# xandercai/JSPSR

Measured on AMD Instinct MI355X. Metric: Mpixels/sec fwd+bwd, JSPSR x8 on 512^2 DEM tiles, higher is better.
Workload: dtype bf16; 1 GPU; jspsr_r8_img_msk (image+mask guided, 43.87M params), 8 x 512x512 tiles per GPU, train step (fwd + L1/L2/Sobel loss + bwd + grad all-reduce + AdamW); storage policy: bf16 activations / gradients / MFMA operands, fp32 accumulation, BatchNorm statistics, master weights and optimizer, and the generator head (affinity logits + offsets) kept as fp32 planes; tiles_per_gpu=8, tile=512, global_tiles=8, parallelism=dp1, step_mode=eager

## Files before the change

jspsr_amd/csrc/conv.hip:

```cpp
#include "conv_igemm.h"

#include <cstdlib>
#include <type_traits>

namespace {

using namespace jspsr;

constexpr int NT = 256;
constexpr int NCH = 8;
template <typename T> struct Elem;
template <> struct Elem<float> { static constexpr int EPC = 4; };
template <> struct Elem<__bf16> { static constexpr int EPC = 8; };

template <typename T> struct Mma;
template <> struct Mma<float> {
  static constexpr int BLK = 32, ROWP = 144, NE = 16, SUB = NCH / 2, SUBB = 32;
  using acc_t = f32x16;
  static __device__ __forceinline__ int frag_row(int lane) { return lane & 31; }
  static __device__ __forceinline__ int frag_chunk(int lane) { return lane >> 5; }
  static __device__ __forceinline__ int acc_row(int lane, int e) { return (e & 3) + 8 * (e >> 2) + 4 * (lane >> 5); }
  static __device__ __forceinline__ int acc_col(int lane) { return lane & 31; }
};
template <> struct Mma<__bf16> {
// ... 661 lines not shown
      if (s + 1 < M::SUB) __builtin_amdgcn_sched_group_barrier(0x100, NR, 0);
      __builtin_amdgcn_sched_group_barrier(0x008, NM, 0);
    }
  };
  auto step = [&](auto CUR, auto NXT) {
    load_b(CUR);
    const bool first_tap = (cty == 0 && ctx == 0), more = cchunk + 1 < nchunks;
    if (first_tap && more) load_patch(cchunk + 1);
    CL_STAMP(0);
    compute(CUR);
    CL_STAMP(1);
    const bool last_tap = (cty == g.nty - 1 && ctx == g.ntx - 1);
    if (last_tap && more) {
      __syncthreads();
      store_patch();
    }
    CL_STAMP(2);
    store_b(NXT, NXT);
    CL_STAMP(3);
    __syncthreads();
    CL_STAMP(4);
    if (++ctx == g.ntx) { ctx = 0; if (++cty == g.nty) { cty = 0; ++cchunk; } }
  };
  CL_STAMP3(5);
  if (KT > 0) {
    load_patch(0);
    load_b(S0{});
    load_b(S1{});
    CL_STAMP3(6);
    store_patch();
    store_b(S0{}, S0{});
  }
  CL_STAMP3(7);
  __syncthreads();
#ifdef CONVLAB_STAMPS
  CL_NOW(cl_last);
  cl_first = cl_last;
#endif
#ifdef CONVLAB_PRIO
  if ((blockIdx.x >> CONVLAB_PRIO) & 1) __builtin_amdgcn_s_setprio(1);
#endif
  int kt = 0;
  for (; kt + 1 < KT; kt += 2) {
    step(S0{}, S1{});
    step(S1{}, S0{});
  }
  if (kt < KT) step(S0{}, S1{});

#ifdef CONVLAB_STAMPS
  unsigned long long cl_loop;
  CL_NOW(cl_loop);
  cl_last = cl_loop;
#endif
  auto out_pixel = [&](int row) -> long long {
    const int y = ty0 + (row >> 4), x = tx0 + ((row + rot * (row >> 4)) & (TLW - 1));
    const int oy = y * g.oy_mul + g.oy_add, ox = x * g.ox_mul + g.ox_add;
    return (y < g.MH && x < g.MW && oy < g.OH && ox < g.OW) ? ((long long)bimg * g.OH + oy) * g.OW + ox : -1;
  };
  if (stats) {
    if constexpr (BM == 128) {
      stats_epilogue<M, MI, NI, WGM, WTM, WTN, BN>(acc, stats, smem, mt, g.Cout, n0, wm, wn, lane, out_pixel);
    } else {
      const int tty8 = (g.MH + 7) / 8;
      const int r1 = (bimg * tty8 + 2 * tyi) * ttx + txi;
      const int r2 = (2 * tyi + 1 < tty8) ? r1 + ttx : -1;
      stats_epilogue<M, MI, NI, WGM, WTM, WTN, BN>(acc, stats, smem, r1, g.Cout, n0, wm, wn, lane, out_pixel, r2);
    }
  }
  float bv[NI], sv[NI];
  int ncol[NI];
  const bool relu_first = g.relu && !g.addend, relu_last = g.relu && g.addend;
#pragma unroll
  for (int ni = 0; ni < NI; ++ni) {
    ncol[ni] = n0 + wn * WTN + ni * BLK + lc;
    bv[ni] = (bias && ncol[ni] < g.Cout) ? bias[ncol[ni]] : 0.f;
    sv[ni] = (g.scale && ncol[ni] < g.Cout) ? g.scale[ncol[ni]] : 1.f;
  }
  constexpr int OPITCH = BN * (int)sizeof(T) + 16;
  char* Os = smem;
  const bool vec_ok = (g.Cout % EPC == 0) && ((g.out_cstride * (int)sizeof(T)) % 16 == 0) &&
                      (((g.out_coff + n0) * (int)sizeof(T)) % 16 == 0) &&
                      ((reinterpret_cast<uintptr_t>(out) & 15u) == 0) &&
                      (!g.addend || (((reinterpret_cast<uintptr_t>(g.addend) & 15u) == 0) &&
                                     ((g.add_cstride * (int)sizeof(T)) % 16 == 0) && ((n0 * (int)sizeof(T)) % 16 == 0)));
  if (vec_ok) {
    constexpr int CPRO = BN * (int)sizeof(T) / 16;
    constexpr int O_IT = BM * CPRO / NTH, OB = O_IT <= 8 ? O_IT : 8;
    static_assert(BM * CPRO % NTH == 0 && O_IT % OB == 0, "epilogue rows");
    long long ooff[OB];
    uint4 areg[OB];
    uint4 zreg[OB];
    const int oy_t = ty0 * g.oy_mul + g.oy_add, ox_t = tx0 * g.ox_mul + g.ox_add, ystep = g.oy_mul * g.OW;
    const long long pix_t = ((long long)bimg * g.OH + oy_t) * g.OW + ox_t;
    const unsigned ocs = (unsigned)g.out_cstride * (unsigned)sizeof(T), acs = (unsigned)g.add_cstride * (unsigned)sizeof(T);
    const long long obase_t = pix_t * ocs, abase_t = pix_t * acs + n0 * (long long)sizeof(T);
    const unsigned zcs = (unsigned)g.red_cstride * (unsigned)sizeof(T);
    const long long zbase_t = pix_t * zcs + n0 * (long long)sizeof(T);
    const bool inside = ty0 + TLH <= g.MH && tx0 + TLW <= g.MW && oy_t + (TLH - 1) * g.oy_mul < g.OH &&
                        ox_t + (TLW - 1) * g.ox_mul < g.OW && n0 + BN <= g.Cout;
    auto plan_pieces = [&](int j0) __attribute__((always_inline)) {
#pragma unroll
      for (int j = 0; j < OB; ++j) {
        const int i = tid + (j0 + j) * NTH, row = i / CPRO, c16 = i % CPRO;
        const int dy = row >> 4, dx = (row + rot * dy) & (TLW - 1);
        const unsigned dpix = (unsigned)(dy * ystep + dx * g.ox_mul);
        bool ok = true;
        if (!inside)
          ok = ty0 + dy < g.MH && tx0 + dx < g.MW && oy_t + dy * g.oy_mul < g.OH && ox_t + dx * g.ox_mul < g.OW &&
               n0 + c16 * EPC < g.Cout;
        ooff[j] = ok ? obase_t + (long long)((unsigned long long)dpix * ocs) + c16 * 16 : -1;
        if (g.addend) {
          areg[j] = make_uint4(0, 0, 0, 0);
          if (ok)
            areg[j] = *reinterpret_cast<const uint4*>(static_cast<const char*>(g.addend) + abase_t +
                                                      (long long)((unsigned long long)dpix * acs) + c16 * 16);
        }
        if (g.red_out) {
          zreg[j] = make_uint4(0, 0, 0, 0);
          if (ok)
            zreg[j] = *reinterpret_cast<const uint4*>(static_cast<const char*>(g.red_x) + zbase_t +
                                                      (long long)((unsigned long long)dpix * zcs) + c16 * 16);
        }
      }
    };
    float rs1[EPC], rs2[EPC], rpa[EPC], rpb[EPC], rpi[EPC], rpm[EPC];
    if (g.red_out) {
      static_assert(NTH % CPRO == 0, "a thread's pieces share their channels");
      const int cc = n0 + (tid % CPRO) * EPC;
#pragma unroll
      for (int e2 = 0; e2 < EPC; ++e2) {
        const bool in_c = cc + e2 < g.Cout;
        rs1[e2] = rs2[e2] = 0.f;
        rpa[e2] = in_c ? g.red_par[cc + e2] : 0.f;
        rpb[e2] = in_c ? g.red_par[g.Cout + cc + e2] : 0.f;
        rpi[e2] = in_c ? g.red_par[2 * g.Cout + cc + e2] : 0.f;
        rpm[e2] = in_c ? g.red_par[3 * g.Cout + cc + e2] : 0.f;
      }
    }
    plan_pieces(0);
#pragma unroll
    for (int mi = 0; mi < MI; ++mi)
#pragma unroll
      for (int e = 0; e < M::NE; ++e) {
        const int row = wm * WTM + mi * BLK + M::acc_row(lane, e);
#pragma unroll
        for (int ni = 0; ni < NI; ++ni) {
          float v = acc[mi][ni][e] * sv[ni] + bv[ni];
          if (relu_first) v = fmaxf(v, 0.f);
          *reinterpret_cast<T*>(Os + row * OPITCH + (wn * WTN + ni * BLK + lc) * (int)sizeof(T)) = (T)v;
        }
      }
    CL_STAMP3(0);
    __syncthreads();
    CL_STAMP3(1);
    char* const obase = reinterpret_cast<char*>(out + g.out_coff + n0);
#pragma unroll
    for (int j0 = 0; j0 < O_IT; j0 += OB) {
      if (j0) plan_pieces(j0);
      uint4 ov[OB];
#pragma unroll
      for (int j = 0; j < OB; ++j) {
        const int i = tid + (j0 + j) * NTH, row = i / CPRO, c16 = i % CPRO;
        ov[j] = *reinterpret_cast<const uint4*>(Os + row * OPITCH + c16 * 16);
      }
      CL_STAMP3(2);
#pragma unroll
      for (int j = 0; j < OB; ++j) {
        if (ooff[j] < 0) continue;
        uint4 v = ov[j];
        if (g.addend) v = add_packed<T>(v, areg[j]);
        if (relu_last) v = relu_packed<T>(v);
        *reinterpret_cast<uint4*>(obase + ooff[j]) = v;
        if (g.red_out) {
          float dv[EPC], zv[EPC];
          unpack_chunk<T>(v, dv);
          unpack_chunk<T>(zreg[j], zv);
#pragma unroll
          for (int e2 = 0; e2 < EPC; ++e2) {
            const float dz = rpa[e2] * zv[e2] + rpb[e2] > 0.f ? dv[e2] : 0.f;
            rs1[e2] += dz;
            rs2[e2] += dz * (zv[e2] * rpi[e2] + rpm[e2]);
          }
        }
      }
    }
    if (g.red_out) {
      __syncthreads();
      float* red = reinterpret_cast<float*>(smem);
#pragma unroll
      for (int e2 = 0; e2 < EPC; ++e2) {
        red[tid * 2 * EPC + e2] = rs1[e2];
        red[tid * 2 * EPC + EPC + e2] = rs2[e2];
      }
      __syncthreads();
      int r1 = mt, r2 = -1;
      if constexpr (BM != 128) {
        const int tty8 = (g.MH + 7) / 8;
        r1 = (bimg * tty8 + 2 * tyi) * ttx + txi;
        r2 = (2 * tyi + 1 < tty8) ? r1 + ttx : -1;
      }
      for (int i = tid; i < 2 * BN; i += NTH) {
        const int which = i / BN, col = i % BN;
        if (n0 + col >= g.Cout) continue;
        const int cg_ = col / EPC, e2 = col % EPC;
        float tsum = 0.f;
        for (int k2 = 0; k2 < NTH / CPRO; ++k2) tsum += red[(cg_ + CPRO * k2) * 2 * EPC + which * EPC + e2];
        g.red_out[((size_t)r1 * 2 + which) * g.Cout + n0 + col] = tsum;
        if (r2 >= 0) g.red_out[((size_t)r2 * 2 + which) * g.Cout + n0 + col] = 0.f;
      }
    }
  } else {
#pragma unroll
    for (int mi = 0; mi < MI; ++mi)
#pragma unroll
      for (int e = 0; e < M::NE; ++e) {
        const int row = wm * WTM + mi * BLK + M::acc_row(lane, e);
        const long long opix = out_pixel(row);
        if (opix < 0) continue;
        T* orow = out + opix * g.out_cstride + g.out_coff;
#pragma unroll
        for (int ni = 0; ni < NI; ++ni) {
          if (ncol[ni] >= g.Cout) continue;
          float v = acc[mi][ni][e] * sv[ni] + bv[ni];
          if (relu_first) v = fmaxf(v, 0.f);
          if (g.addend) v = (float)(T)v + (float)static_cast<const T*>(g.addend)[opix * g.add_cstride + ncol[ni]];
          if (relu_last) v = fmaxf(v, 0.f);
          orow[ncol[ni]] = (T)v;
        }
      }
  }
#ifdef CONVLAB_STAMPS
  if ((tid & 63) == 0) {
    unsigned long long end_;
    CL_NOW(end_);
    unsigned long long* o = convlab_stamp + (size_t)((blockIdx.x * (NTH / 64) + (tid >> 6)) % CONVLAB_SLOTS) * 16;
    for (int i = 0; i < 4; ++i) o[i] = cl_stamp[i] + (i == 3 ? cl_stamp[4] : 0);
    o[4] = cl_first - cl_entry;
    o[5] = cl_loop - cl_first;
    o[6] = end_ - cl_loop;
    for (int i = 5; i < 8; ++i) o[3 + i] = cl_stamp[i];
    o[11] = cl_stamp[4];
    o[7] = (unsigned long long)KT;
  }
#endif
}

template <typename T, int BM, int BN, int WGM, int WGN>
int launch_patch(const void* in, const void* wgt, const float* bias, void* out, float* stats, const ConvGeom& g, hipStream_t s) {
  constexpr int NTH = 64 * WGM * WGN, TLW = 16, TLH = BM / TLW, MAXPIX = patch_it(BM, NTH) * NTH / NCH;
  const long long nblk = (long long)g.B * ((g.MH + TLH - 1) / TLH) * ((g.MW + TLW - 1) / TLW) * ((g.Cout + BN - 1) / BN);
  if (nblk > 0x7fffffffLL || (long long)TLH * g.oy_mul * g.OW + (long long)TLW * g.ox_mul > 0x7fffffffLL)
    return fail(JSPSR_EINVAL, "conv: grid too large");
  constexpr int ROWB = Mma<T>::ROWP;
  const size_t lds_stage = (size_t)MAXPIX * ROWB + 2 * BN * ROWB, lds_out = (size_t)BM * (BN * sizeof(T) + 16);
  const size_t lds = lds_stage > lds_out ? lds_stage : lds_out;
  ConvGeom gk = g;
  gk.fd_ntn = make_fastdiv((unsigned)((g.Cout + BN - 1) / BN));
  gk.fd_ttx = make_fastdiv((unsigned)((g.MW + TLW - 1) / TLW));
  gk.fd_tty = make_fastdiv((unsigned)((g.MH + TLH - 1) / TLH));
  auto kern = conv_patch_kernel<T, BM, BN, WGM, WGN>;
  static bool attr_set = false;
  if (!attr_set) {
    (void)hipFuncSetAttribute(reinterpret_cast<const void*>(kern), hipFuncAttributeMaxDynamicSharedMemorySize, (int)lds);
    attr_set = true;
  }
  hipLaunchKernelGGL(kern, dim3((unsigned)nblk), dim3(NTH), lds, s, static_cast<const T*>(in), static_cast<const T*>(wgt),
                     bias, static_cast<T*>(out), stats, gk);
  return check_launch(BM == 256 ? (BN == 64 ? "conv_patch_16x16" : "conv_patch_16x16x128") : "conv_patch");
}

template <typename T, int BM, int BN, int WGM, int WGN, int NBUF>
int launch_cfg(const void* in, const void* wgt, const float* bias, void* out, float* stats, const ConvGeom& g, hipStream_t s) {
  if ((long long)g.B * g.MH * g.MW <= 0) return JSPSR_OK;
  constexpr int TLW = 16, TLH = BM / TLW;
  const long long nblk = (long long)g.B * ((g.MH + TLH - 1) / TLH) * ((g.MW + TLW - 1) / TLW) * ((g.Cout + BN - 1) / BN);
  if (nblk > 0x7fffffffLL) return fail(JSPSR_EINVAL, "conv: grid too large");
  constexpr int ROWB = IgemmMma<T, NBUF>::ROWP;
  const size_t lds_stage = NBUF * (BM + BN) * ROWB, lds_out = (size_t)BM * (BN * sizeof(T) + 16);
  const size_t lds = lds_stage > lds_out ? lds_stage : lds_out;
  constexpr int BK = NCH * Elem<T>::EPC;
  static bool attr_set = false;
  if (!attr_set) {
    (void)hipFuncSetAttribute(reinterpret_cast<const void*>(conv_igemm_kernel<T, BM, BN, WGM, WGN, true, NBUF>),
                              hipFuncAttributeMaxDynamicSharedMemorySize, (int)lds);
    (void)hipFuncSetAttribute(reinterpret_cast<const void*>(conv_igemm_kernel<T, BM, BN, WGM, WGN, false, NBUF>),
                              hipFuncAttributeMaxDynamicSharedMemorySize, (int)lds);
    attr_set = true;
  }
  if (g.Cin % BK == 0)
    hipLaunchKernelGGL((conv_igemm_kernel<T, BM, BN, WGM, WGN, true, NBUF>), dim3((unsigned)nblk), dim3(NT), lds, s,
                       static_cast<const T*>(in), static_cast<const T*>(wgt), bias, static_cast<T*>(out), stats, g);
  else
    hipLaunchKernelGGL((conv_igemm_kernel<T, BM, BN, WGM, WGN, false, NBUF>), dim3((unsigned)nblk), dim3(NT), lds, s,
                       static_cast<const T*>(in), static_cast<const T*>(wgt), bias, static_cast<T*>(out), stats, g);
  return check_launch("conv_igemm");
}

template <typename T>
int launch(const void* in, const void* wgt, const float* bias, void* out, float* stats, const ConvGeom& g, hipStream_t s) {
  static const int no_patch = [] { const char* e = getenv("JSPSR_CONV_NOPATCH"); return e ? atoi(e) : 0; }();
  constexpr int BKT = NCH * Elem<T>::EPC;
  if constexpr (sizeof(T) == 2)
  {
    if (conv64_resident_ok(g, in, wgt, bias, out)) return launch_conv64_resident(in, wgt, bias, out, stats, g, s);
    if (conv128_resident_ok(g, in, wgt, bias, out)) return launch_conv128_resident(in, wgt, bias, out, stats, g, s);
  }
  if ((!no_patch || g.in_affine) && g.iy_mul == 1 && g.ix_mul == 1 && g.nty >= 1 && g.ntx >= 1 && g.nty <= 3 && g.ntx <= 3 &&
      g.nty * g.ntx > 1 && g.Cin % BKT == 0 && (long long)(g.IW + 20) * 12 * g.in_cstride * (long long)sizeof(T) < 0xE0000000LL) {
    static const int tall = [] { const char* e = getenv("JSPSR_CONV_TALL"); return e ? atoi(e) : 1; }();
    const long long tiles16 = (long long)g.B * ((g.MH + 15) / 16) * ((g.MW + 15) / 16);
    if (g.Cout > 64) {
      if (tall == 2 && tiles16 * ((g.Cout + 127) / 128) >= 512) return launch_patch<T, 256, 128, 4, 2>(in, wgt, bias, out, stats, g, s);
      if (tall && tall != 4 && tiles16 * ((g.Cout + 63) / 64) >= 1024) return launch_patch<T, 256, 64, 4, 1>(in, wgt, bias, out, stats, g, s);
      return launch_patch<T, 128, 128, 2, 2>(in, wgt, bias, out, stats, g, s);
    }
    if (g.Cout > 32) {
      if (tall && tiles16 >= 1024) return launch_patch<T, 256, 64, 4, 1>(in, wgt, bias, out, stats, g, s);
      return launch_patch<T, 128, 64, 2, 2>(in, wgt, bias, out, stats, g, s);
    }
    return launch_patch<T, 128, 32, 4, 1>(in, wgt, bias, out, stats, g, s);
  }
  if (g.red_out) return fail(JSPSR_EINVAL, "conv2d_dgrad: the fused BatchNorm-backward reduce needs the patch kernel (jspsr_conv2d_dgrad_reduce_ok)");
  if (g.in_affine) return fail(JSPSR_EINVAL, "conv2d_forward: in_affine needs the patch kernel (stride 1, 2..9 taps, Cin a multiple of %d): ask jspsr_conv2d_in_affine_ok first", BKT);
  static const int nbuf_env = [] { const char* e = getenv("JSPSR_CONV_NBUF"); return e ? atoi(e) : 0; }();
  const int nbuf_narrow = nbuf_env ? nbuf_env : ((long long)g.nty * g.ntx * g.Cin <= 1152 ? 1 : 2);
  if (g.Cout > 64) return launch_cfg<T, 128, 128, 2, 2, 2>(in, wgt, bias, out, stats, g, s);
  if (nbuf_narrow == 2) {
    if (g.Cout > 32) return launch_cfg<T, 128, 64, 2, 2, 2>(in, wgt, bias, out, stats, g, s);
    return launch_cfg<T, 128, 32, 4, 1, 2>(in, wgt, bias, out, stats, g, s);
  }
  if (g.Cout > 32) return launch_cfg<T, 128, 64, 2, 2, 1>(in, wgt, bias, out, stats, g, s);
  return launch_cfg<T, 128, 32, 4, 1, 1>(in, wgt, bias, out, stats, g, s);
}

int check_common(int dtype, const void* a, const void* w, const void* o, int cin, int cs_in, int co_in,
                 int cs_out, int co_out, int cout, const char* what) {
  if (dtype != JSPSR_F32 && dtype != JSPSR_BF16) return fail(JSPSR_EINVAL, "%s: dtype must be JSPSR_F32 or JSPSR_BF16", what);
  if (!a || !w || !o) return fail(JSPSR_EINVAL, "%s: null pointer", what);
  const int epc = dtype == JSPSR_F32 ? 4 : 8;
  if (cin <= 0 || cin % epc || cs_in % epc || co_in % epc || cs_in < co_in + cin)
    return fail(JSPSR_EINVAL, "%s: gathered channels (C=%d pitch=%d off=%d) must be multiples of %d", what, cin, cs_in, co_in, epc);
  if (cout <= 0 || cs_out < co_out + cout) return fail(JSPSR_EINVAL, "%s: bad output channel slice", what);
  if (!aligned16(a) || !aligned16(w)) return fail(JSPSR_EALIGN, "%s: input/weight pointers must be 16-byte aligned", what);
  return JSPSR_OK;
}

template <typename T>
__global__ void pack_weight_kernel(const float* __restrict__ w, T* __restrict__ out, int O, int I, int KH, int KW,
                                   int mode, int Cpad, long long total) {
  for (long long idx = blockIdx.x * (long long)blockDim.x + threadIdx.x; idx < total;
       idx += (long long)gridDim.x * blockDim.x) {
    const int c = (int)(idx % Cpad);
    long long r = idx / Cpad;
    const int kx = (int)(r % KW); r /= KW;
    const int ky = (int)(r % KH); r /= KH;
    const int n = (int)r;
    float v = 0.f;
    if (mode == 0) { if (c < I) v = w[(((size_t)n * I + c) * KH + ky) * KW + kx]; }
    else           { if (c < O) v = w[(((size_t)c * I + n) * KH + ky) * KW + kx]; }
    out[idx] = (T)v;
  }
}

constexpr int PACK_CHUNK = 2048;
__global__ __launch_bounds__(256) void pack_weights_multi_kernel(const jspsr_pack_desc* __restrict__ descs, int n) {
  int lo = 0, hi = n - 1;
  const long long b = blockIdx.x;
  while (lo < hi) {
    const int mid = (lo + hi + 1) >> 1;
    if (descs[mid].start <= b) lo = mid; else hi = mid - 1;
  }
  const jspsr_pack_desc d = descs[lo];
  const long long l0 = (b - d.start) * PACK_CHUNK;
  const float* __restrict__ w = d.w;
#pragma unroll
  for (int k = 0; k < PACK_CHUNK / 256; ++k) {
    const long long l = l0 + k * 256 + threadIdx.x;
    if (l >= d.total) break;
    const int c = (int)(l % d.c_pad);
    long long r = l / d.c_pad;
    const int kx = (int)(r % d.KW); r /= d.KW;
    const int ky = (int)(r % d.KH); r /= d.KH;
    const int nn = (int)r;
    float v = 0.f;
    if (d.mode == 0) { if (c < d.I) v = w[(((size_t)nn * d.I + c) * d.KH + ky) * d.KW + kx]; }
    else             { if (c < d.O) v = w[(((size_t)c * d.I + nn) * d.KH + ky) * d.KW + kx]; }
    if (d.dtype == JSPSR_F32) static_cast<float*>(d.out)[l] = v;
    else static_cast<__bf16*>(d.out)[l] = (__bf16)v;
  }
}

}

extern "C" int jspsr_pack_weights_multi(const jspsr_pack_desc* descs, int n, long long total_blocks, jspsr_stream_t stream) {
  if (!descs || n <= 0 || total_blocks <= 0 || total_blocks > 0x7fffffffLL) return fail(JSPSR_EINVAL, "pack_weights_multi: bad arguments");
  hipLaunchKernelGGL(pack_weights_multi_kernel, dim3((unsigned)total_blocks), dim3(256), 0, static_cast<hipStream_t>(stream), descs, n);
  return check_launch("pack_weights_multi");
}

extern "C" int jspsr_pack_chunk(void) { return PACK_CHUNK; }

extern "C" int jspsr_pack_weight(int dtype, const float* w, void* packed, int O, int I, int KH, int KW,
                                 int mode, int c_pad, jspsr_stream_t stream) {
  if (!w || !packed || O <= 0 || I <= 0 || KH <= 0 || KW <= 0 || (mode != 0 && mode != 1))
    return fail(JSPSR_EINVAL, "pack_weight: bad arguments");
  const int C = mode == 0 ? I : O, N = mode == 0 ? O : I;
  if (c_pad < C) return fail(JSPSR_EINVAL, "pack_weight: c_pad %d < %d", c_pad, C);
  const long long total = (long long)N * KH * KW * c_pad;
  const int blocks = (int)((total + 255) / 256 < 4096 ? (total + 255) / 256 : 4096);
  hipStream_t s = static_cast<hipStream_t>(stream);
  if (dtype == JSPSR_F32)
    hipLaunchKernelGGL(pack_weight_kernel<float>, dim3(blocks), dim3(256), 0, s, w, static_cast<float*>(packed), O, I, KH, KW, mode, c_pad, total);
  else if (dtype == JSPSR_BF16)
    hipLaunchKernelGGL(pack_weight_kernel<__bf16>, dim3(blocks), dim3(256), 0, s, w, static_cast<__bf16*>(packed), O, I, KH, KW, mode, c_pad, total);
  else
    return fail(JSPSR_EINVAL, "pack_weight: bad dtype");
  return check_launch("pack_weight");
}

extern "C" int jspsr_conv2d_stats_rows(int B, int OH, int OW) {
  if (B <= 0 || OH <= 0 || OW <= 0) return 0;
  return B * ((OH + 7) / 8) * ((OW + 15) / 16);
}

extern "C" int jspsr_conv2d_forward(int dtype, const void* in, const void* wpack, const float* bias, void* out,
                                    int B, int IH, int IW, int Cin, int in_cstride, int in_coff, int Cout,
                                    int out_cstride, int out_coff, int KH, int KW, int stride, int pad, int relu,
                                    float* stats, const float* scale, const void* addend, int add_cstride,
                                    const float* in_affine, int in_relu, jspsr_stream_t stream) {
  if (int e = check_common(dtype, in, wpack, out, Cin, in_cstride, in_coff, out_cstride, out_coff, Cout, "conv2d_forward")) return e;
  if (in_affine && !aligned16(in_affine)) return fail(JSPSR_EALIGN, "conv2d_forward: in_affine must be 16-byte aligned");
  if (addend && add_cstride < Cout) return fail(JSPSR_EINVAL, "conv2d_forward: addend pitch %d < %d channels", add_cstride, Cout);
  if (B <= 0 || IH <= 0 || IW <= 0 || KH <= 0 || KW <= 0 || stride <= 0 || pad < 0)
    return fail(JSPSR_EINVAL, "conv2d_forward: bad geometry");
  ConvGeom g{};
  g.B = B; g.IH = IH; g.IW = IW; g.Cin = Cin;
  g.OH = (IH + 2 * pad - KH) / stride + 1;
  g.OW = (IW + 2 * pad - KW) / stride + 1;
  if (g.OH <= 0 || g.OW <= 0) return fail(JSPSR_EINVAL, "conv2d_forward: empty output");
  g.Cout = Cout; g.in_cstride = in_cstride; g.in_coff = in_coff; g.out_cstride = out_cstride; g.out_coff = out_coff;
  g.MH = g.OH; g.MW = g.OW;
  g.iy_mul = stride; g.iy_add = -pad; g.ix_mul = stride; g.ix_add = -pad; g.sign = 1;
  g.nty = KH; g.ntx = KW; g.ky0 = 0; g.kx0 = 0; g.kstep = 1; g.KH = KH; g.KW = KW;
  g.oy_mul = 1; g.oy_add = 0; g.ox_mul = 1; g.ox_add = 0; g.relu = relu;
  g.accumulate = getenv("JSPSR_CONV_NOXCD") ? 1 : 0;
  hipStream_t s = static_cast<hipStream_t>(stream);
  if (stats && (bias || relu || scale || addend))
    return fail(JSPSR_EINVAL, "conv2d_forward: statistics are taken from the raw accumulators (no bias / scale / addend / ReLU)");
  g.scale = scale; g.addend = addend; g.add_cstride = add_cstride;
  g.in_affine = in_affine; g.in_relu = in_relu;
  return dtype == JSPSR_F32 ? launch<float>(in, wpack, bias, out, stats, g, s) : launch<__bf16>(in, wpack, bias, out, stats, g, s);
}

extern "C" int jspsr_conv2d_in_affine_ok(int dtype, int Cin, int KH, int KW, int stride) {
  const int bk = NCH * (dtype == JSPSR_F32 ? 4 : 8);
  return (dtype == JSPSR_F32 || dtype == JSPSR_BF16) && stride == 1 && KH >= 1 && KW >= 1 && KH <= 3 && KW <= 3 && KH * KW > 1 &&
         Cin > 0 && Cin % bk == 0;
}

extern "C" int jspsr_conv2d_dgrad_reduce_ok(int dtype, int B, int IH, int IW, int Cg, int Cin, int KH, int KW, int stride, int pad) {
  if (dtype != JSPSR_F32 && dtype != JSPSR_BF16) return 0;
  static const int off = [] { const char* e = getenv("JSPSR_BN_REDUCE_FUSE"); return e && atoi(e) == 0; }();
  if (off) return 0;
  const int epc = dtype == JSPSR_F32 ? 4 : 8, bkt = NCH * epc;
  if (KH != 3 || KW != 3 || stride != 1 || pad != 1 || Cg <= 0 || Cg % bkt || Cin <= 0 || Cin % epc || B <= 0 || IH <= 0 || IW <= 0) return 0;
  static const int no_patch = [] { const char* e = getenv("JSPSR_CONV_NOPATCH"); return e ? atoi(e) : 0; }();
  if (no_patch) return 0;
  if (dtype == JSPSR_BF16 && Cg == 64 && Cin == 64) {
    static const int resident = [] { const char* e = getenv("JSPSR_CONV_RESIDENT"); return e ? atoi(e) : 1; }();
    static const int min_tiles = [] { const char* e = getenv("JSPSR_CONV_RESIDENT_MIN"); return e ? atoi(e) : 512; }();
    if (resident && (long long)B * ((IH + 15) / 16) * ((IW + 15) / 16) >= min_tiles) return 0;
  }
  return 1;
}

extern "C" int jspsr_conv2d_dgrad(int dtype, const void* gout, const void* wpack_t, const float* bias, void* gin,
                                  int B, int OH, int OW, int Cg, int g_cstride, int g_coff, int IH, int IW,
                                  int Cin, int in_cstride, int in_coff, int KH, int KW, int stride, int pad,
                                  int relu, const void* addend, int add_cstride, const float* scale,
                                  const void* red_x, int red_cstride, const float* red_par, float* red_out,
                                  jspsr_stream_t stream) {
  if (int e = check_common(dtype, gout, wpack_t, gin, Cg, g_cstride, g_coff, in_cstride, in_coff, Cin, "conv2d_dgrad")) return e;
  if (addend && add_cstride < Cin) return fail(JSPSR_EINVAL, "conv2d_dgrad: addend pitch %d < %d channels", add_cstride, Cin);
  if (red_out) {
    if (!red_x || !red_par || !jspsr_conv2d_dgrad_reduce_ok(dtype, B, IH, IW, Cg, Cin, KH, KW, stride, pad))
      return fail(JSPSR_EINVAL, "conv2d_dgrad: the fused BatchNorm-backward reduce needs jspsr_conv2d_dgrad_reduce_ok(...) != 0");
    const int epc = dtype == JSPSR_F32 ? 4 : 8;
    if (red_cstride < Cin || red_cstride % epc || in_cstride % epc || in_coff % epc || !aligned16(red_x) || !aligned16(gin) ||
        (addend && (!aligned16(addend) || add_cstride % epc)))
      return fail(JSPSR_EALIGN, "conv2d_dgrad: fused reduce needs 16-byte pieces (pitches / offsets multiples of %d, aligned tensors)", epc);
  }
  if (B <= 0 || OH <= 0 || OW <= 0 || IH <= 0 || IW <= 0 || KH <= 0 || KW <= 0 || stride <= 0 || pad < 0)
    return fail(JSPSR_EINVAL, "conv2d_dgrad: bad geometry");
  hipStream_t s = static_cast<hipStream_t>(stream);
  for (int py = 0; py < stride; ++py)
    for (int px = 0; px < stride; ++px) {
      ConvGeom g{};
      g.B = B; g.IH = OH; g.IW = OW; g.Cin = Cg;
      g.OH = IH; g.OW = IW; g.Cout = Cin;
      g.in_cstride = g_cstride; g.in_coff = g_coff; g.out_cstride = in_cstride; g.out_coff = in_coff;
      g.MH = (IH - py + stride - 1) / stride;
      g.MW = (IW - px + stride - 1) / stride;
      if (g.MH <= 0 || g.MW <= 0) continue;
      g.ky0 = (py + pad) % stride; g.kx0 = (px + pad) % stride; g.kstep = stride;
      g.nty = g.ky0 < KH ? (KH - g.ky0 + stride - 1) / stride : 0;
      g.ntx = g.kx0 < KW ? (KW - g.kx0 + stride - 1) / stride : 0;
      if (g.nty == 0 || g.ntx == 0) g.nty = g.ntx = 0;
      g.iy_mul = 1; g.iy_add = (py + pad - g.ky0) / stride; g.ix_mul = 1; g.ix_add = (px + pad - g.kx0) / stride;
      g.sign = -1; g.KH = KH; g.KW = KW;
      g.oy_mul = stride; g.oy_add = py; g.ox_mul = stride; g.ox_add = px; g.relu = relu;
      g.addend = addend; g.add_cstride = add_cstride; g.scale = scale;
      g.red_x = red_x; g.red_cstride = red_cstride; g.red_par = red_par; g.red_out = red_out;
      const int e = dtype == JSPSR_F32 ? launch<float>(gout, wpack_t, bias, gin, nullptr, g, s)
                                       : launch<__bf16>(gout, wpack_t, bias, gin, nullptr, g, s);
      if (e) return e;
    }
  return JSPSR_OK;
}

#ifdef CONVLAB_STAMPS
extern "C" int jspsr_lab_conv_stamps(unsigned long long* out16, int reset) {
  static unsigned long long host[CONVLAB_SLOTS * 16];
  if (hipMemcpyFromSymbol(host, HIP_SYMBOL(convlab_stamp), sizeof(host)) != hipSuccess) return 1;
  for (int i = 0; i < 16; ++i) out16[i] = 0;
  for (int r = 0; r < CONVLAB_SLOTS; ++r)
    if (host[r * 16 + 7]) { for (int i = 0; i < 16; ++i) out16[i] += host[r * 16 + i]; }
  if (reset) { for (size_t i = 0; i < sizeof(host) / 8; ++i) host[i] = 0; if (hipMemcpyToSymbol(HIP_SYMBOL(convlab_stamp), host, sizeof(host)) != hipSuccess) return 1; }
  return 0;
}
#endif
```

jspsr_amd/csrc/conv128.hip:

```cpp
#include "conv_igemm.h"

#include <atomic>

#include <cstdlib>
#include <type_traits>

namespace {

using namespace jspsr;

constexpr int Q_NTH = 256;
constexpr int Q_TH = 8, Q_TW = 16;
constexpr int Q_PH = Q_TH + 2, Q_PW = Q_TW + 2, Q_NPIX = Q_PH * Q_PW;
constexpr int Q_PIXB = 256;
constexpr int Q_PATCHB = Q_NPIX * Q_PIXB;
constexpr int Q_PIECES = Q_PATCHB / 1024;
static_assert(Q_PIECES * 1024 == Q_PATCHB, "whole pieces");
constexpr int Q_NP = (Q_PIECES + 3) / 4;
constexpr int Q_BUF1 = 65536;
constexpr int Q_XCHB = 16384;
constexpr int Q_OFF_RED = Q_PATCHB + Q_XCHB;
static_assert(Q_OFF_RED + 2048 <= Q_BUF1, "the first 64 KiB hold patch 0, inbox 0 and the fold");
constexpr int Q_OFF_RUN = Q_OFF_RED + 2048;
static_assert(Q_OFF_RUN + 16 <= Q_BUF1, "run starts inside the first 64 KiB");
constexpr int Q_RUN = 4;
constexpr int Q_OFF_DUMP = Q_BUF1 + Q_PATCHB + 3 * Q_XCHB;
constexpr int Q_OFF_PAR = Q_OFF_DUMP + 1024;
constexpr int Q_LDS = Q_OFF_PAR + 1024;
static_assert(Q_LDS <= 163840, "LDS of one CU");
constexpr int Q_ROWS4 = 4 * Q_PW * Q_PIXB;
#ifndef K2Q_LA
#define K2Q_LA 4
#endif
#ifndef K2Q_DMA_MODE
#define K2Q_DMA_MODE 1
#endif
#ifndef K2Q_LD_EVERY
#define K2Q_LD_EVERY 9
#endif
#ifndef K2Q_LD_DIST
#define K2Q_LD_DIST 27
#endif
#ifndef K2Q_DMA_EVERY
#define K2Q_DMA_EVERY 6
#endif
constexpr int Q_NK = 144, Q_LAH = K2Q_LA;

__device__ __forceinline__ int inbox_off(int wave) { return wave == 0 ? Q_PATCHB : Q_BUF1 + Q_PATCHB + (wave - 1) * Q_XCHB; }

template <int SH, int N>
__device__ __forceinline__ void row_sum(float (&v)[N]) {
#pragma unroll
  for (int c = 0; c < N; ++c)
    v[c] += __builtin_bit_cast(float, __builtin_amdgcn_update_dpp(0, __builtin_bit_cast(int, v[c]), 0x120 + SH, 0xf, 0xf, false));
}

template <int B, int E, typename F>
__device__ __forceinline__ void static_for(F&& f) {
  if constexpr (B < E) {
    f(std::integral_constant<int, B>{});
    static_for<B + 1, E>(f);
  }
}

template <bool FIRST, bool WA>
__device__ __forceinline__ void mfma4(f32x4& c0, f32x4& c1, f32x4& c2, f32x4& c3, const i32x4& w0, const i32x4& w1, const i32x4& w2,
                                      const i32x4& w3, const i32x4& b) {
#define K2Q_MFMA4(OUT, CC, WC)                                                                                           \
  asm volatile("v_mfma_f32_16x16x32_bf16 %0, %4, %8, " CC "0\n\tv_mfma_f32_16x16x32_bf16 %1, %5, %8, " CC "1\n\t"        \
               "v_mfma_f32_16x16x32_bf16 %2, %6, %8, " CC "2\n\tv_mfma_f32_16x16x32_bf16 %3, %7, %8, " CC "3"             \
               : OUT(c0), OUT(c1), OUT(c2), OUT(c3) : WC(w0), WC(w1), WC(w2), WC(w3), "v"(b))
  if constexpr (FIRST) {
    if constexpr (WA)
      asm volatile("v_mfma_f32_16x16x32_bf16 %0, %4, %8, 0\n\tv_mfma_f32_16x16x32_bf16 %1, %5, %8, 0\n\t"
                   "v_mfma_f32_16x16x32_bf16 %2, %6, %8, 0\n\tv_mfma_f32_16x16x32_bf16 %3, %7, %8, 0"
                   : "=&v"(c0), "=&v"(c1), "=&v"(c2), "=&v"(c3) : "a"(w0), "a"(w1), "a"(w2), "a"(w3), "v"(b));
    else
      asm volatile("v_mfma_f32_16x16x32_bf16 %0, %4, %8, 0\n\tv_mfma_f32_16x16x32_bf16 %1, %5, %8, 0\n\t"
                   "v_mfma_f32_16x16x32_bf16 %2, %6, %8, 0\n\tv_mfma_f32_16x16x32_bf16 %3, %7, %8, 0"
                   : "=&v"(c0), "=&v"(c1), "=&v"(c2), "=&v"(c3) : "v"(w0), "v"(w1), "v"(w2), "v"(w3), "v"(b));
  } else {
    if constexpr (WA) K2Q_MFMA4("+v", "%", "a");
    else K2Q_MFMA4("+v", "%", "v");
  }
#undef K2Q_MFMA4
}

typedef const i32x4 __attribute__((address_space(3)))* lds_frag_t;

struct QTile { int bimg, tyi, txi; };
struct QSrc { i32x4 desc; __amdgpu_buffer_rsrc_t rsrc; int oy0, ox0; bool interior; };

template <int SIGN, int MODE, int KH>
__device__ __forceinline__ void conv128_body(const __bf16* __restrict__ in, const __bf16* __restrict__ wgt, const float* __restrict__ bias,
                                             __bf16* __restrict__ out, float* __restrict__ stats, const ConvGeom& g, int ntiles, unsigned* __restrict__ ticket, char* smem) {
  constexpr bool STATS = MODE == 1, AFFINE = MODE == 2;
  const int tid = threadIdx.x, wave = __builtin_amdgcn_readfirstlane(tid >> 6), lane = tid & 63;
  const int cg = wave & 1;
  const int n = lane & 15, q = lane >> 4;
  const int ttx = (g.MW + Q_TW - 1) / Q_TW, tty = (g.MH + Q_TH - 1) / Q_TH;
  const int G = gridDim.x;
  const unsigned lds0 = (unsigned)(size_t)(lptr_t)smem;
  if (lds0 != 0) __builtin_trap();
  const int v = xcd_contiguous(blockIdx.x, G);

  i32x4 breg[9][2][4];
#pragma unroll
  for (int cb = 0; cb < 4; ++cb) {
    const int ch = 64 * cg + 32 * (cb >> 1) + 8 * (n >> 2) + 4 * (cb & 1) + (n & 3);
    const char* wrow = reinterpret_cast<const char*>(wgt) + (size_t)ch * (9 * 128 * 2) + (64 * KH + 8 * q) * 2;
#pragma unroll
    for (int t = 0; t < 9; ++t)
#pragma unroll
      for (int s = 0; s < 2; ++s) breg[t][s][cb] = *reinterpret_cast<const i32x4*>(wrow + t * 256 + s * 64);
  }

  const int dGx = G % ttx, dGy = (G / ttx) % tty, dGb = G / (ttx * tty);
  auto advance = [&](QTile c) {
    c.txi += dGx;
    int carry = c.txi >= ttx;
    c.txi -= carry ? ttx : 0;
    c.tyi += dGy + carry;
    carry = c.tyi >= tty;
    c.tyi -= carry ? tty : 0;
    c.bimg += dGb + carry;
    return c;
  };

  const int pix_bytes = g.in_cstride * 2;
  constexpr int back = SIGN < 0 ? 2 : 0;
  auto patch_src = [&](QTile tc, bool more) {
    QSrc p;
    p.oy0 = tc.tyi * Q_TH + g.iy_add - back;
    p.ox0 = tc.txi * Q_TW + g.ix_add - back;
    const long long opix0 = ((long long)tc.bimg * g.IH + p.oy0) * g.IW + p.ox0;
    const unsigned long long b64 = reinterpret_cast<unsigned long long>(in) + (opix0 * g.in_cstride + g.in_coff) * 2;
    p.desc = i32x4{(int)(unsigned)b64, (int)((unsigned)(b64 >> 32) & 0xffffu), more ? (int)0xFFFFFF00u : 0, 0x00020000};
    p.interior = p.oy0 >= 0 && p.ox0 >= 0 && p.oy0 + Q_PH <= g.IH && p.ox0 + Q_PW <= g.IW;
    p.rsrc = __builtin_amdgcn_make_buffer_rsrc(reinterpret_cast<char*>(b64), 0, more ? 0xFFFFFF00u : 0u, 0x00020000);
    return p;
  };
  const int p0lane = 4 * wave + q;
  const unsigned swz16 = (unsigned)((n ^ (2 * (p0lane & 7))) << 4);
  unsigned dsrc[Q_NP];
#pragma unroll
  for (int i = 0; i < Q_NP; ++i) {
    const int P = p0lane + 16 * i, py = P / Q_PW, px = P - py * Q_PW;
    dsrc[i] = (unsigned)((py * g.IW + px) * pix_bytes) + swz16;
  }
  struct PieceXY { int py, px; unsigned off; };
  auto piece_xy = [&](int i) __attribute__((always_inline)) {
    int p0 = p0lane;
    asm volatile("" : "+v"(p0));
    const int P = p0 + 16 * i;
    PieceXY c;
    c.py = (int)(__umul24(P, 3641) >> 16);
    unsigned t = __umul24(c.py, Q_PW);
    asm("" : "+v"(t));
    c.px = P - (int)t;
    unsigned t2 = __umul24(c.py, g.IW);
    asm("" : "+v"(t2));
    c.off = t2 + (unsigned)c.px;
    return c;
  };
  auto piece_src = [&](const QSrc& p, const PieceXY& c) __attribute__((always_inline)) {
    unsigned b = __umul24(c.off, pix_bytes);
    asm("" : "+v"(b));
    unsigned src = b + swz16;
    src = (unsigned)(p.oy0 + c.py) < (unsigned)g.IH ? src : 0xFFFFFFF0u;
    src = (unsigned)(p.ox0 + c.px) < (unsigned)g.IW ? src : 0xFFFFFFF0u;
    return src;
  };
  auto piece_dst = [&](unsigned bufoff, int i) __attribute__((always_inline)) {
#ifdef K2Q_LAB_TODUMP
    return (unsigned)Q_OFF_DUMP;
#endif
    return (wave + 4 * i < Q_PIECES) ? bufoff + (unsigned)(wave + 4 * i) * 1024u : (unsigned)Q_OFF_DUMP;
  };
  auto issue_piece = [&](const QSrc& p, unsigned bufoff, int i) __attribute__((always_inline)) {
    unsigned src = dsrc[i];
    if (!p.interior) src = piece_src(p, piece_xy(i));
    const unsigned dst = lds0 + piece_dst(bufoff, i);
#if defined(K2Q_LAB_NOISSUE)
    asm volatile("" : : "s"(dst), "v"(src), "s"(p.desc));
#elif defined(K2Q_LAB_OOB)
    asm volatile("s_mov_b32 m0, %0\n\ts_nop 4\n\tbuffer_load_dwordx4 %1, %2, 0 offen lds" : : "s"(dst), "v"(src | 0xF0000000u), "s"(p.desc));
#else
    asm volatile("s_mov_b32 m0, %0\n\ts_nop 4\n\tbuffer_load_dwordx4 %1, %2, 0 offen lds" : : "s"(dst), "v"(src), "s"(p.desc));
#endif
  };

  unsigned abase[4][3];
#pragma unroll
  for (int b = 0; b < 4; ++b)
#pragma unroll
    for (int tx = 0; tx < 3; ++tx)
      abase[b][tx] = (unsigned)((Q_PW * b + tx + n) * Q_PIXB + (((8 * KH + q) ^ (2 * ((2 * b + tx + n) & 7))) << 4));

  auto prefetch_addend = [&](QTile tc) __attribute__((always_inline)) {
    const int y = tc.tyi * Q_TH + 4 * KH + q, x = tc.txi * Q_TW + n;
    const unsigned off = (y < g.MH && x < g.MW) ? (unsigned)(y * g.OW + x) * (unsigned)(g.add_cstride * 2) : 0xFFFFFFF0u;
    const unsigned long long b64 = reinterpret_cast<unsigned long long>(g.addend) + ((long long)tc.bimg * g.OH * g.OW * g.add_cstride + 64 * cg) * 2;
    const i32x4 d = {(int)(unsigned)b64, (int)((unsigned)(b64 >> 32) & 0xffffu), g.addend ? (int)0xFFFFFF00u : 0, 0x00020000};
    asm volatile("s_mov_b32 m0, %0\n\ts_nop 4\n\tbuffer_load_dwordx4 %1, %2, 0 offen lds" : : "s"(lds0 + (unsigned)Q_OFF_DUMP), "v"(off), "s"(d));
  };

  char* const give = smem + inbox_off(wave ^ 2) + lane * 16;
  const char* const take = smem + inbox_off(wave) + lane * 16;
  f32x4 acc[8][4];
  auto meet = [&]() __attribute__((always_inline)) {
    asm volatile("s_nop 15\n\ts_nop 15" ::: "memory");
#pragma unroll
    for (int i = 0; i < 4; ++i)
#pragma unroll
      for (int cb = 0; cb < 4; ++cb) *reinterpret_cast<f32x4*>(give + (i * 4 + cb) * 1024) = acc[4 * (1 - KH) + i][cb];
    asm volatile("s_waitcnt lgkmcnt(0)" ::: "memory");
    __builtin_amdgcn_s_barrier();
    asm volatile("" ::: "memory");
#pragma unroll
    for (int i = 0; i < 4; ++i)
#pragma unroll
      for (int cb = 0; cb < 4; ++cb) acc[4 * KH + i][cb] = *reinterpret_cast<const f32x4*>(take + (i * 4 + cb) * 1024);
  };

  auto mfma_tile = [&](const QSrc& nxt, unsigned nbufoff, QTile tc) __attribute__((always_inline)) {
    i32x4 a[Q_LAH];
    constexpr int NSTG = (K2Q_LD_DIST + K2Q_LD_EVERY - 1) / K2Q_LD_EVERY;
    u32x4 stg[NSTG];
    static_for<0, Q_NK + Q_LAH>([&](auto K) __attribute__((always_inline)) {
      constexpr int k = decltype(K)::value;
      if constexpr (k >= Q_LAH) {
        constexpr int kk = k - Q_LAH, half = kk / 72, st = (kk % 72) >> 2, tap = st >> 1, s = st & 1;
        constexpr int r = (half == 0 ? 4 * (1 - KH) : 4 * KH) + (kk & 3);
        if constexpr (kk == 72) meet();
        mfma4<(half == 0 && st == 0), (tap < 8)>(acc[r][0], acc[r][1], acc[r][2], acc[r][3], breg[tap][s][0], breg[tap][s][1], breg[tap][s][2],
                                                 breg[tap][s][3], a[kk % Q_LAH]);
      }
      if constexpr (k < Q_NK) {
        constexpr int half = k / 72, st = (k % 72) >> 2, tap = st >> 1, s = st & 1;
        constexpr int r = (half == 0 ? 4 * (1 - KH) : 4 * KH) + (k & 3);
        constexpr int ty = SIGN > 0 ? tap / 3 : 2 - tap / 3, tx = SIGN > 0 ? tap % 3 : 2 - tap % 3;
        constexpr int R = r + ty;
        a[k % Q_LAH] = *reinterpret_cast<lds_frag_t>((abase[R & 3][tx] ^ (unsigned)(s * 64)) + (unsigned)((R >> 2) * Q_ROWS4));
        if constexpr (K2Q_DMA_MODE == 1 && k % K2Q_DMA_EVERY == 2 && k / K2Q_DMA_EVERY < Q_NP) issue_piece(nxt, nbufoff, k / K2Q_DMA_EVERY);
        if constexpr (!STATS && k == 1) prefetch_addend(tc);
        if constexpr (K2Q_DMA_MODE == 3) {
          constexpr int LD = K2Q_LD_EVERY, WD = K2Q_LD_DIST;
          static_assert(2 + LD * (Q_NP - 1) + WD < Q_NK, "the last piece is written inside the loop");
          if constexpr (k >= 2 + WD && (k - 2 - WD) % LD == 0 && (k - 2 - WD) / LD < Q_NP) {
            constexpr int j = (k - 2 - WD) / LD;
            *reinterpret_cast<u32x4*>(smem + piece_dst(nbufoff, j) + lane * 16) = stg[j % NSTG];
          }
          if constexpr (k >= 2 && (k - 2) % LD == 0 && (k - 2) / LD < Q_NP) {
            constexpr int j = (k - 2) / LD;
            stg[j % NSTG] = __builtin_amdgcn_raw_buffer_load_b128(nxt.rsrc, piece_src(nxt, piece_xy(j)), 0, 0);
          }
        }
      }
    });
    asm volatile("s_nop 15\n\ts_nop 15" ::: "memory");
  };

  const bool relu_first = g.relu && !g.addend, relu_last = g.relu && g.addend;
  float* const red = reinterpret_cast<float*>(smem + Q_OFF_RED);
  auto out_desc = [&](int bimg) {
    const unsigned long long b64 = reinterpret_cast<unsigned long long>(out) + ((long long)bimg * g.OH * g.OW * g.out_cstride + g.out_coff + 64 * cg) * 2;
    return __builtin_amdgcn_make_buffer_rsrc(reinterpret_cast<char*>(b64), 0, 0xFFFFFF00u, 0x00020000);
  };
  auto add_desc = [&](int bimg) {
    const unsigned long long b64 = reinterpret_cast<unsigned long long>(g.addend) + ((long long)bimg * g.OH * g.OW * g.add_cstride + 64 * cg) * 2;
    return __builtin_amdgcn_make_buffer_rsrc(reinterpret_cast<char*>(b64), 0, g.addend ? 0xFFFFFF00u : 0u, 0x00020000);
  };

  auto epilogue = [&](QTile tc) __attribute__((always_inline)) {
    const int ty0 = tc.tyi * Q_TH + 4 * KH, x = tc.txi * Q_TW + n;
    const __amdgpu_buffer_rsrc_t orsrc = out_desc(tc.bimg), adrsrc = add_desc(tc.bimg);
    unsigned ooff[4], aoff[4];
    bool inside[4];
#pragma unroll
    for (int i = 0; i < 4; ++i) {
      const int y = ty0 + i;
      inside[i] = y < g.MH && x < g.MW;
      const unsigned pix = (unsigned)(y * g.OW + x);
      ooff[i] = inside[i] ? pix * (unsigned)(g.out_cstride * 2) + q * 16u : 0xFFFFFFF0u;
      aoff[i] = inside[i] ? pix * (unsigned)(g.add_cstride * 2) + q * 16u : 0xFFFFFFF0u;
    }
    if constexpr (STATS) {
      if (stats) {
        const bool whole = tc.tyi * Q_TH + Q_TH <= g.MH && tc.txi * Q_TW + Q_TW <= g.MW;
#pragma unroll
        for (int h = 0; h < 2; ++h) {
          float s1[8], s2[8];
#pragma unroll
          for (int c = 0; c < 8; ++c) { s1[c] = 0.f; s2[c] = 0.f; }
          if (whole) {
#pragma unroll
            for (int i = 0; i < 4; ++i)
#pragma unroll
              for (int c = 0; c < 8; ++c) {
                const float a0 = acc[4 * KH + i][2 * h + (c >> 2)][c & 3];
                s1[c] += a0;
                s2[c] = __builtin_fmaf(a0, a0, s2[c]);
              }
          } else {
#pragma unroll
            for (int i = 0; i < 4; ++i) {
              const float m = inside[i] ? 1.f : 0.f;
#pragma unroll
              for (int c = 0; c < 8; ++c) {
                const float a0 = acc[4 * KH + i][2 * h + (c >> 2)][c & 3] * m;
                s1[c] += a0;
                s2[c] = __builtin_fmaf(a0, a0, s2[c]);
              }
            }
          }
          row_sum<8>(s1); row_sum<8>(s2);
          row_sum<4>(s1); row_sum<4>(s2);
          row_sum<2>(s1); row_sum<2>(s2);
          row_sum<1>(s1); row_sum<1>(s2);
          if (n == 0) {
            float* r1 = red + (KH * 2 + 0) * 128 + 64 * cg + 32 * h + 8 * q;
            float* r2 = red + (KH * 2 + 1) * 128 + 64 * cg + 32 * h + 8 * q;
            *reinterpret_cast<f32x4*>(r1) = f32x4{s1[0], s1[1], s1[2], s1[3]};
            *reinterpret_cast<f32x4*>(r1 + 4) = f32x4{s1[4], s1[5], s1[6], s1[7]};
            *reinterpret_cast<f32x4*>(r2) = f32x4{s2[0], s2[1], s2[2], s2[3]};
            *reinterpret_cast<f32x4*>(r2 + 4) = f32x4{s2[4], s2[5], s2[6], s2[7]};
          }
        }
      }
    }
    if constexpr (AFFINE) {
#pragma unroll
      for (int h = 0; h < 2; ++h) {
        const float* tab = reinterpret_cast<const float*>(smem + Q_OFF_PAR) + 64 * cg + 32 * h + 8 * q;
#pragma unroll
        for (int u = 0; u < 2; ++u) {
          const f32x4 s4 = *reinterpret_cast<const f32x4*>(tab + 4 * u), b4 = *reinterpret_cast<const f32x4*>(tab + 128 + 4 * u);
#pragma unroll
          for (int i = 0; i < 4; ++i)
#pragma unroll
            for (int j = 0; j < 4; ++j) acc[4 * KH + i][2 * h + u][j] = acc[4 * KH + i][2 * h + u][j] * s4[j] + b4[j];
        }
      }
    }
    if (!STATS && g.addend) {
      u32x4 av[4][2];
#pragma unroll
      for (int i = 0; i < 4; ++i)
#pragma unroll
        for (int h = 0; h < 2; ++h) av[i][h] = __builtin_amdgcn_raw_buffer_load_b128(adrsrc, aoff[i], h * 64, 0);
#pragma unroll
      for (int i = 0; i < 4; ++i)
#pragma unroll
        for (int h = 0; h < 2; ++h) {
          const f32x4 lo = acc[4 * KH + i][2 * h], hi = acc[4 * KH + i][2 * h + 1];
          const u32x4 o = {pack_bf16(lo[0], lo[1]), pack_bf16(lo[2], lo[3]), pack_bf16(hi[0], hi[1]), pack_bf16(hi[2], hi[3])};
          __builtin_amdgcn_raw_buffer_store_b128(add_bf16x8(o, av[i][h], relu_last), orsrc, ooff[i], h * 64, 0);
        }
    } else {
      if (!STATS && relu_first) {
#pragma unroll
        for (int i = 0; i < 4; ++i)
#pragma unroll
          for (int cb = 0; cb < 4; ++cb)
#pragma unroll
            for (int j = 0; j < 4; ++j) acc[4 * KH + i][cb][j] = relu_bits(acc[4 * KH + i][cb][j]);
      }
#pragma unroll
      for (int i = 0; i < 4; ++i)
#pragma unroll
        for (int h = 0; h < 2; ++h) {
          const f32x4 lo = acc[4 * KH + i][2 * h], hi = acc[4 * KH + i][2 * h + 1];
          const u32x4 o = {pack_bf16(lo[0], lo[1]), pack_bf16(lo[2], lo[3]), pack_bf16(hi[0], hi[1]), pack_bf16(hi[2], hi[3])};
          __builtin_amdgcn_raw_buffer_store_b128(o, orsrc, ooff[i], h * 64, 0);
        }
    }
  };
  auto flush_stats = [&](QTile tc) __attribute__((always_inline)) {
    const int which = tid >> 7, col = tid & 127;
    stats[((size_t)((tc.bimg * tty + tc.tyi) * ttx + tc.txi) * 2 + which) * 128 + col] = red[which * 128 + col] + red[(2 + which) * 128 + col];
  };

  if constexpr (AFFINE) {
    reinterpret_cast<float*>(smem + Q_OFF_PAR)[tid] = tid < 128 ? (g.scale ? g.scale[tid] : 1.f) : (bias ? bias[tid - 128] : 0.f);
  }
  const bool dyn = ticket != nullptr;
  int* const s_run = reinterpret_cast<int*>(smem + Q_OFF_RUN);
  if (dyn) {
    if (tid == 0) {
      s_run[0] = (int)__hip_atomic_fetch_add(ticket, (unsigned)Q_RUN, __ATOMIC_RELAXED, __HIP_MEMORY_SCOPE_AGENT);
      s_run[1] = (int)__hip_atomic_fetch_add(ticket, (unsigned)Q_RUN, __ATOMIC_RELAXED, __HIP_MEMORY_SCOPE_AGENT);
    }
    __syncthreads();
  }
  auto tile_of = [&](int t_) { return QTile{(t_ / ttx) / tty, (t_ / ttx) % tty, t_ % ttx}; };
  int t = dyn ? s_run[0] : v, it = 0;
  int krun = 0, nrun = 0;
  unsigned pend = 0;
  int pend_slot = -1;
  QTile tcur = tile_of(t < ntiles ? t : 0), tprev = tcur;
  unsigned bufoff = 0;
  if (t < ntiles) {
    const QSrc p0 = patch_src(tcur, true);
#pragma unroll
    for (int i = 0; i < Q_NP; ++i) issue_piece(p0, 0u, i);
  }
  __builtin_amdgcn_s_waitcnt(0x0F70);
  asm volatile("" ::: "memory");
#ifdef K2Q_STAMPS
  unsigned long long st_bar = 0, st_mfma = 0, st_epi = 0, st_vm = 0, s0, s1;
  const unsigned long long c_begin = __builtin_readcyclecounter(), r_begin = __builtin_amdgcn_s_memrealtime();
#define K2Q_STAMP(acc_) do { s1 = __builtin_readcyclecounter(); acc_ += s1 - s0; s0 = s1; } while (0)
#else
#define K2Q_STAMP(acc_) do { } while (0)
#endif
  for (; t < ntiles; ++it) {
#ifdef K2Q_STAMPS
    s0 = __builtin_readcyclecounter();
#endif
    asm volatile("s_waitcnt lgkmcnt(0)" ::: "memory");
    __builtin_amdgcn_s_barrier();
    asm volatile("" ::: "memory");
    K2Q_STAMP(st_bar);
    if (STATS && stats && it > 0) flush_stats(tprev);
    int tn, kn = 0, nn = nrun;
    QTile tnext;
    if (!dyn) {
      tn = t + G;
      tnext = advance(tcur);
    } else if (krun + 1 < Q_RUN && t + 1 < ntiles) {
      tn = t + 1;
      kn = krun + 1;
      tnext = tcur;
      if (++tnext.txi == ttx) { tnext.txi = 0; if (++tnext.tyi == tty) { tnext.tyi = 0; ++tnext.bimg; } }
    } else {
      nn = nrun + 1;
      tn = s_run[nn & 1];
      tnext = tile_of(tn < ntiles ? tn : 0);
    }
    if (dyn && tid == 0 && krun == 0) {
      asm volatile("s_nop 4\n\tglobal_atomic_add %0, %1, %2, %3 sc0" : "+v"(pend) : "v"(0u), "v"((unsigned)Q_RUN), "s"(ticket));
      pend_slot = nrun & 1;
    }
    const bool more = tn < ntiles;
    const QSrc nxt = patch_src(tnext, more);
    if (K2Q_DMA_MODE == 0) {
#pragma unroll
      for (int i = 0; i < Q_NP; ++i) issue_piece(nxt, bufoff ^ Q_BUF1, i);
    }
    mfma_tile(nxt, bufoff ^ Q_BUF1, tcur);
    K2Q_STAMP(st_mfma);
    epilogue(tcur);
    K2Q_STAMP(st_epi);
#pragma unroll
    for (int b = 0; b < 4; ++b)
#pragma unroll
      for (int tx = 0; tx < 3; ++tx) abase[b][tx] ^= (unsigned)Q_BUF1;
    bufoff ^= Q_BUF1;
    asm volatile("s_waitcnt vmcnt(8)" ::: "memory");
    K2Q_STAMP(st_vm);
    if (dyn && tid == 0 && pend_slot >= 0) { s_run[pend_slot] = (int)pend; pend_slot = -1; }
    tprev = tcur;
    tcur = tnext;
    t = tn; krun = kn; nrun = nn;
  }
#ifdef K2Q_STAMPS
  if (blockIdx.x == 0 && lane == 0 && (wave == 0 || wave == 2) && it > 0) {
    const unsigned long long dc = __builtin_readcyclecounter() - c_begin, dr = __builtin_amdgcn_s_memrealtime() - r_begin;
    printf("K2Q wave %d tiles %d: barrier %llu  tap loop incl. the meeting %llu  epilogue %llu  vmcnt %llu (cycles per tile); clock %.0f MHz\n",
           wave, it, st_bar / it, st_mfma / it, st_epi / it, st_vm / it, 100.0 * (double)dc / (double)dr);
  }
#endif
  if (dyn && tid == 0) {
    __builtin_amdgcn_s_waitcnt(0x0F70);
    const unsigned old = __hip_atomic_fetch_add(ticket + 1, 1u, __ATOMIC_RELAXED, __HIP_MEMORY_SCOPE_AGENT);
    if (old == (unsigned)G - 1u) {
      __hip_atomic_store(ticket, 0u, __ATOMIC_RELAXED, __HIP_MEMORY_SCOPE_AGENT);
      __hip_atomic_store(ticket + 1, 0u, __ATOMIC_RELAXED, __HIP_MEMORY_SCOPE_AGENT);
    }
  }
  if (STATS && stats && it > 0) {
    __syncthreads();
    flush_stats(tprev);
  }
}

template <int SIGN, int MODE>
__global__ __launch_bounds__(Q_NTH) __attribute__((amdgpu_waves_per_eu(1, 1))) void conv128_resident_kernel(
    const __bf16* __restrict__ in, const __bf16* __restrict__ wgt, const float* __restrict__ bias, __bf16* __restrict__ out,
    float* __restrict__ stats, ConvGeom g, int ntiles, unsigned* __restrict__ ticket) {
  extern __shared__ __attribute__((aligned(128))) char smem[];
  if (__builtin_amdgcn_readfirstlane(threadIdx.x >> 7) == 0) conv128_body<SIGN, MODE, 0>(in, wgt, bias, out, stats, g, ntiles, ticket, smem);
  else conv128_body<SIGN, MODE, 1>(in, wgt, bias, out, stats, g, ntiles, ticket, smem);
}

__device__ unsigned k2q_ring[2 * 1024];

unsigned* next_ticket() {
  static unsigned* base = [] {
    void* p = nullptr;
    return hipGetSymbolAddress(&p, HIP_SYMBOL(k2q_ring)) == hipSuccess ? static_cast<unsigned*>(p) : nullptr;
  }();
  static std::atomic<unsigned> n{0};
  return base ? base + 2 * (n.fetch_add(1, std::memory_order_relaxed) % 1024u) : nullptr;
}

template <int SIGN, int MODE>
void launch_k2q(const void* in, const void* wgt, const float* bias, void* out, float* stats, const ConvGeom& g, int ntiles, int grid, hipStream_t s) {
  static bool attr_set = false;
  if (!attr_set) {
    (void)hipFuncSetAttribute(reinterpret_cast<const void*>(conv128_resident_kernel<SIGN, MODE>), hipFuncAttributeMaxDynamicSharedMemorySize, Q_LDS);
    attr_set = true;
  }
  static const int dynq = [] { const char* e = getenv("JSPSR_CONV_DYNQ128"); return e ? atoi(e) : 0; }();
  const int forced = conv_dynq_override();
  unsigned* ticket = ((forced >= 0 ? forced : dynq) && (long long)ntiles >= 4LL * Q_RUN * grid) ? next_ticket() : nullptr;
  hipLaunchKernelGGL((conv128_resident_kernel<SIGN, MODE>), dim3(grid), dim3(Q_NTH), Q_LDS, s, static_cast<const __bf16*>(in),
                     static_cast<const __bf16*>(wgt), bias, static_cast<__bf16*>(out), stats, g, ntiles, ticket);
}

}

namespace jspsr {

bool conv128_resident_ok(const ConvGeom& g, const void* in, const void* wgt, const float* bias, const void* out) {
  static const int enabled = [] { const char* e = getenv("JSPSR_CONV_RESIDENT128"); return e ? atoi(e) : 1; }();
  if (!enabled) return false;
  if (g.Cin != 128 || g.Cout != 128 || g.nty != 3 || g.ntx != 3 || g.KH != 3 || g.KW != 3) return false;
  if (g.iy_mul != 1 || g.ix_mul != 1 || g.oy_mul != 1 || g.ox_mul != 1 || g.oy_add != 0 || g.ox_add != 0) return false;
  if (g.ky0 != 0 || g.kx0 != 0 || g.kstep != 1 || g.in_affine || g.red_out) return false;
  if (bias && !aligned4(bias)) return false;
  if (g.sign < 0 && (bias || g.scale)) return false;
  if (g.in_cstride % 8 || g.in_coff % 8 || g.out_cstride % 8 || g.out_coff % 8) return false;
  if (!aligned16(in) || !aligned16(wgt) || !aligned16(out)) return false;
  if (g.addend && (!aligned16(g.addend) || g.add_cstride % 8)) return false;
  if ((long long)(g.IW + 20) * 12 * g.in_cstride * 2 >= 0x7fffffffLL || g.IW >= (1 << 20) || g.in_cstride >= (1 << 20)) return false;
  if ((long long)g.OH * g.OW * g.out_cstride * 2 >= 0xF0000000LL || (long long)g.OH * g.OW * g.add_cstride * 2 >= 0xF0000000LL)
    return false;
  const long long tiles = (long long)g.B * ((g.MH + Q_TH - 1) / Q_TH) * ((g.MW + Q_TW - 1) / Q_TW);
  static const int min_tiles = [] { const char* e = getenv("JSPSR_CONV_RESIDENT128_MIN"); return e ? atoi(e) : 2048; }();
  return tiles >= min_tiles && tiles < 0x7fffffffLL;
}

int launch_conv128_resident(const void* in, const void* wgt, const float* bias, void* out, float* stats, const ConvGeom& g, hipStream_t s) {
  const int ntiles = g.B * ((g.MH + Q_TH - 1) / Q_TH) * ((g.MW + Q_TW - 1) / Q_TW);
  static int ncu = 0;
  if (!ncu) {
    int dev = 0;
    hipDeviceProp_t p;
    if (hipGetDevice(&dev) != hipSuccess || hipGetDeviceProperties(&p, dev) != hipSuccess) return fail((int)hipErrorInvalidDevice, "conv: device query failed");
    ncu = p.multiProcessorCount > 0 ? p.multiProcessorCount : 256;
  }
  const int grid = ntiles < ncu ? ntiles : ncu;
  static const int trace = [] { const char* e = getenv("JSPSR_CONV_TRACE128"); return e ? atoi(e) : 0; }();
  if (trace)
    fprintf(stderr, "K2q sign %d B %d %dx%d in pitch %d off %d out pitch %d off %d addend %d (pitch %d) relu %d stats %d in %p out %p\n", g.sign, g.B,
            g.MH, g.MW, g.in_cstride, g.in_coff, g.out_cstride, g.out_coff, g.addend != nullptr, g.add_cstride, g.relu, stats != nullptr, in, out);
  const int mode = stats ? 1 : ((bias || g.scale) ? 2 : 0);
  if (g.sign > 0) {
    if (mode == 0) launch_k2q<1, 0>(in, wgt, bias, out, stats, g, ntiles, grid, s);
    else if (mode == 1) launch_k2q<1, 1>(in, wgt, bias, out, stats, g, ntiles, grid, s);
    else launch_k2q<1, 2>(in, wgt, bias, out, stats, g, ntiles, grid, s);
  } else {
    if (mode != 0) return fail(JSPSR_EINVAL, "conv128_resident: the reversed walk has no statistics / affine form");
    launch_k2q<-1, 0>(in, wgt, bias, out, stats, g, ntiles, grid, s);
  }
  return check_launch("conv128_resident");
}

}
```

jspsr_amd/csrc/conv64.hip:

```cpp
#include "conv_igemm.h"

#include <atomic>

#include <cstdlib>
#include <type_traits>

namespace {

using namespace jspsr;

constexpr int R_NTH = 512;
constexpr int R_PW = 18, R_NPIX = R_PW * R_PW;
constexpr int R_PITCH = 144;
constexpr int R_PPP = 7;
constexpr int R_PIECEB = R_PPP * R_PITCH;
constexpr int R_PIECES = (R_NPIX + R_PPP - 1) / R_PPP;
#ifdef K2R_ORDER
constexpr int order_of(bool) { return K2R_ORDER; }
#else
constexpr int order_of(bool stats) { return stats ? 0 : 2; }
#endif
#ifdef K2R_EARLY
constexpr int early_pieces(bool) { return K2R_EARLY; }
#else
constexpr int early_pieces(bool stats) { return stats ? 8 : 6; }
#endif
constexpr int R_PATCHB = R_PIECES * R_PIECEB + 16;
constexpr int R_SCRP = 80;
constexpr int R_SCRB = 64 * R_SCRP;
constexpr int R_OFF_SCR = 2 * R_PATCHB;
constexpr int R_OFF_RED = R_OFF_SCR + 8 * R_SCRB;
constexpr int R_RUNB = 16;
constexpr int R_LDS_STATS = R_OFF_RED + 3 * 4 * 2 * 64 * 4 + R_RUNB;
constexpr int R_LDS_PLAIN = 2 * R_PATCHB + R_RUNB;
constexpr int R_OFF_PAR = 2 * R_PATCHB;
constexpr int R_LDS_AFFINE = R_OFF_PAR + 2 * 64 * 4 + R_RUNB;
constexpr int R_RUN = 4;
#ifndef K2R_LA
#define K2R_LA 4
#endif
constexpr int R_ROT = 14;
constexpr int NK = 72, LA = K2R_LA;

struct Tile { int bimg, tyi, txi; };
struct PatchSrc { i32x4 desc; int oy0, ox0; bool interior; };

template <int SIGN, int MODE>
__global__ __launch_bounds__(R_NTH) void conv64_resident_kernel(const __bf16* __restrict__ in, const __bf16* __restrict__ wgt,
                                                                  const float* __restrict__ bias, __bf16* __restrict__ out,
                                                                  float* __restrict__ stats, ConvGeom g, int ntiles,
                                                                  unsigned* __restrict__ ticket) {
  constexpr bool STATS = MODE == 1, AFFINE = MODE == 2;
  constexpr int LDSB = MODE == 1 ? R_LDS_STATS : (MODE == 2 ? R_LDS_AFFINE : R_LDS_PLAIN);
  extern __shared__ __attribute__((aligned(128))) char smem[];
  const int tid = threadIdx.x, wave = __builtin_amdgcn_readfirstlane(tid >> 6), lane = tid & 63;
  const int wm = (wave >> 1) & 3, wn = wave & 1;
  const int lr = lane & 31, lh = lane >> 5;
  const int ttx = (g.MW + 15) >> 4, tty = (g.MH + 15) >> 4;
  const int G = gridDim.x;
  const unsigned lds0 = (unsigned)(size_t)(lptr_t)smem;
  const int v = xcd_contiguous(blockIdx.x, G);
  const bool late = wave >= 4;
  constexpr int ORDER = order_of(STATS), R_PE = early_pieces(STATS), R_PL = (R_PIECES - 4 * R_PE + 3) / 4;
  constexpr int R_PIT = R_PE > R_PL ? R_PE : R_PL;

  bf16x8 breg[9][4];
  {
    const char* wrow = reinterpret_cast<const char*>(wgt) + (size_t)(wn * 32 + lr) * (9 * 64 * 2) + lh * 16;
#pragma unroll
    for (int t = 0; t < 9; ++t)
#pragma unroll
      for (int s = 0; s < 4; ++s) breg[t][s] = *reinterpret_cast<const bf16x8*>(wrow + t * 128 + s * 32);
  }

  const int dGx = G % ttx, dGy = (G / ttx) % tty, dGb = G / (ttx * tty);
  auto advance = [&](Tile c) {
    c.txi += dGx;
    int carry = c.txi >= ttx;
    c.txi -= carry ? ttx : 0;
    c.tyi += dGy + carry;
    carry = c.tyi >= tty;
    c.tyi -= carry ? tty : 0;
    c.bimg += dGb + carry;
    return c;
  };

  const int pix_bytes = g.in_cstride * 2;
  const int lpix = lane / 9, lp16 = (lane - 9 * lpix) * 16;
  const int back = SIGN < 0 ? 2 : 0;
  const int piece0 = late ? 4 * R_PE + (wave - 4) : wave, npiece = late ? R_PL : R_PE;
  unsigned dsrc[R_PIT];
#pragma unroll
  for (int i = 0; i < R_PIT; ++i) {
    const int P = (piece0 + 4 * i) * R_PPP + lpix;
    const int py = P / R_PW, px = P - py * R_PW;
    dsrc[i] = (lp16 < 128 && P < R_NPIX) ? (unsigned)((py * g.IW + px) * pix_bytes + lp16) : 0xFFFFFFF0u;
  }
  auto patch_src = [&](Tile tc) {
    PatchSrc p;
    p.oy0 = tc.tyi * 16 + g.iy_add - back;
    p.ox0 = tc.txi * 16 + g.ix_add - back;
    const long long opix0 = ((long long)tc.bimg * g.IH + p.oy0) * g.IW + p.ox0;
    const unsigned long long b64 = reinterpret_cast<unsigned long long>(in) + (opix0 * g.in_cstride + g.in_coff) * 2;
    p.desc = i32x4{(int)(unsigned)b64, (int)((unsigned)(b64 >> 32) & 0xffffu), (int)0xFFFFFF00u, 0x00020000};
    p.interior = p.oy0 >= 0 && p.ox0 >= 0 && p.oy0 + R_PW <= g.IH && p.ox0 + R_PW <= g.IW;
    return p;
  };
  auto issue_patch = [&](const PatchSrc& p, int buf) __attribute__((always_inline)) {
#pragma unroll
    for (int i = 0; i < R_PIT; ++i) {
      if (i < npiece && piece0 + 4 * i < R_PIECES) {
        unsigned src = dsrc[i];
        if (!p.interior) {
          int lpix_ = lpix;
          asm volatile("" : "+v"(lpix_));
          const int P = (piece0 + 4 * i) * R_PPP + lpix_;
          const int py = (int)(__umul24(P, 3641) >> 16), px = P - (int)__umul24(py, R_PW);
          const bool in_img = (unsigned)(p.oy0 + py) < (unsigned)g.IH && (unsigned)(p.ox0 + px) < (unsigned)g.IW;
          src = in_img ? src : 0xFFFFFFF0u;
        }
        const unsigned dst = lds0 + buf * R_PATCHB + (piece0 + 4 * i) * R_PIECEB;
        asm volatile("s_mov_b32 m0, %0\n\ts_nop 0\n\tbuffer_load_dwordx4 %1, %2, 0 offen lds" : : "s"(dst), "v"(src), "s"(p.desc));
      }
    }
  };

  int a_base[2];
#pragma unroll
  for (int mi = 0; mi < 2; ++mi) {
    const int R = wm * 64 + mi * 32 + lr, dy = R >> 4;
    a_base[mi] = (dy * R_PW + ((R + R_ROT * dy) & 15)) * R_PITCH + lh * 16;
  }

  f32x16 acc[2];
  auto mfma_tile = [&](int buf) __attribute__((always_inline)) {
#pragma unroll
    for (int mi = 0; mi < 2; ++mi)
#pragma unroll
      for (int e = 0; e < 16; ++e) acc[mi][e] = 0.f;
    const char* const pa0 = smem + buf * R_PATCHB + a_base[0];
    const char* const pa1 = smem + buf * R_PATCHB + a_base[1];
    bf16x8 a[LA];
#pragma unroll
    for (int k = 0; k < NK + LA; ++k) {
      if (k >= LA) {
        const int kk = k - LA, tap = kk >> 3, s = (kk >> 1) & 3, mi = kk & 1;
        if (STATS) acc[mi] = __builtin_amdgcn_mfma_f32_32x32x16_bf16(a[kk % LA], breg[tap][s], acc[mi], 0, 0, 0);
        else       acc[mi] = __builtin_amdgcn_mfma_f32_32x32x16_bf16(breg[tap][s], a[kk % LA], acc[mi], 0, 0, 0);
      }
      if (k < NK) {
        const int tap = k >> 3, s = (k >> 1) & 3, mi = k & 1;
        const int tp = (tap / 3) * R_PW + tap % 3;
        a[k % LA] = *reinterpret_cast<const bf16x8*>((mi ? pa1 : pa0) + (SIGN > 0 ? tp : 2 * R_PW + 2 - tp) * R_PITCH + s * 32);
      }
    }
    __builtin_amdgcn_sched_group_barrier(0x100, LA, 0);
#pragma unroll
    for (int k = 0; k < NK; ++k) {
      __builtin_amdgcn_sched_group_barrier(0x008, 1, 0);
      if (k + LA < NK) __builtin_amdgcn_sched_group_barrier(0x100, 1, 0);
    }
  };

  const bool relu_first = g.relu && !g.addend, relu_last = g.relu && g.addend;
  char* const scr = smem + R_OFF_SCR + wave * R_SCRB;
  float* const red = reinterpret_cast<float*>(smem + R_OFF_RED);
  const int ncol = wn * 32 + lr;
  const int tty8 = (g.MH + 7) >> 3;

  auto flush_stats = [&](Tile tc, int par) __attribute__((always_inline)) {
    if (tid < 256) {
      const int half = tid >> 7, which = (tid >> 6) & 1, col = tid & 63;
      const int row = 2 * tc.tyi + half;
      if (row < tty8) {
        const float* r0 = red + ((par * 4 + 2 * half) * 2 + which) * 64 + col;
        stats[((size_t)((tc.bimg * tty8 + row) * ttx + tc.txi) * 2 + which) * 64 + col] = r0[0] + r0[2 * 64];
      }
    }
  };

  auto out_desc = [&](int bimg) {
    const unsigned long long b64 = reinterpret_cast<unsigned long long>(out) + ((long long)bimg * g.OH * g.OW * g.out_cstride + g.out_coff + wn * 32) * 2;
    return __builtin_amdgcn_make_buffer_rsrc(reinterpret_cast<char*>(b64), 0, 0xFFFFFF00u, 0x00020000);
  };
  auto add_desc = [&](int bimg) {
    const unsigned long long b64 = reinterpret_cast<unsigned long long>(g.addend) + ((long long)bimg * g.OH * g.OW * g.add_cstride + wn * 32) * 2;
    return __builtin_amdgcn_make_buffer_rsrc(reinterpret_cast<char*>(b64), 0, g.addend ? 0xFFFFFF00u : 0u, 0x00020000);
  };

  auto epilogue_stats = [&](Tile tc, int par) __attribute__((always_inline)) {
    const int ty0 = tc.tyi * 16, tx0 = tc.txi * 16;
    const bool whole = ty0 + 16 <= g.MH && tx0 + 16 <= g.MW;
    if (stats) {
      float s = 0.f, q = 0.f;
      if (whole) {
        f32x2 s2 = {0.f, 0.f}, q2 = {0.f, 0.f};
#pragma unroll
        for (int mi = 0; mi < 2; ++mi)
#pragma unroll
          for (int e = 0; e < 16; e += 2) {
            const f32x2 a2 = {acc[mi][e], acc[mi][e + 1]};
            s2 += a2;
            q2 = __builtin_elementwise_fma(a2, a2, q2);
          }
        s = s2[0] + s2[1];
        q = q2[0] + q2[1];
      } else {
        int lh4 = 4 * lh;
        asm volatile("" : "+v"(lh4));
#pragma unroll
        for (int mi = 0; mi < 2; ++mi)
#pragma unroll
          for (int e = 0; e < 16; ++e) {
            const int R = wm * 64 + mi * 32 + (e & 3) + 8 * (e >> 2) + lh4, dy = R >> 4;
            const int y = ty0 + dy, x = tx0 + ((R + R_ROT * dy) & 15);
            if (y < g.MH && x < g.MW) {
              const float a0 = acc[mi][e];
              s += a0;
              q += a0 * a0;
            }
          }
      }
      s += __shfl_xor(s, 32, 64);
      q += __shfl_xor(q, 32, 64);
      if (lh == 0) {
        red[((par * 4 + wm) * 2 + 0) * 64 + ncol] = s;
        red[((par * 4 + wm) * 2 + 1) * 64 + ncol] = q;
      }
    }
#pragma unroll
    for (int mi = 0; mi < 2; ++mi)
#pragma unroll
      for (int e = 0; e < 16; ++e) {
        const int row = mi * 32 + (e & 3) + 8 * (e >> 2) + 4 * lh;
        const float o = acc[mi][e];
        *reinterpret_cast<__bf16*>(scr + row * R_SCRP + lr * 2) = (__bf16)o;
      }
    asm volatile("s_waitcnt lgkmcnt(0)" ::: "memory");
    const int c16 = lane & 3, prow = lane >> 2;
    const __amdgpu_buffer_rsrc_t orsrc = out_desc(tc.bimg), adrsrc = add_desc(tc.bimg);
    unsigned ooff[4], aoff[4];
#pragma unroll
    for (int j = 0; j < 4; ++j) {
      const int dy = wm * 4 + j;
      const int y = ty0 + dy, x = tx0 + ((prow + R_ROT * dy) & 15);
      const bool inside = whole || (y < g.MH && x < g.MW);
      const unsigned pix = (unsigned)(y * g.OW + x);
      ooff[j] = inside ? pix * (unsigned)(g.out_cstride * 2) + c16 * 16u : 0xFFFFFFF0u;
      aoff[j] = inside ? pix * (unsigned)(g.add_cstride * 2) + c16 * 16u : 0xFFFFFFF0u;
    }
    if (g.addend) {
      u32x4 av[4];
#pragma unroll
      for (int j = 0; j < 4; ++j) av[j] = __builtin_amdgcn_raw_buffer_load_b128(adrsrc, aoff[j], 0, 0);
#pragma unroll
      for (int j = 0; j < 4; ++j) {
        const u32x4 o = *reinterpret_cast<const u32x4*>(scr + (j * 16 + prow) * R_SCRP + c16 * 16);
        __builtin_amdgcn_raw_buffer_store_b128(add_bf16x8(o, av[j], relu_last), orsrc, ooff[j], 0, 0);
      }
    } else {
#pragma unroll
      for (int j = 0; j < 4; ++j) {
        const u32x4 o = *reinterpret_cast<const u32x4*>(scr + (j * 16 + prow) * R_SCRP + c16 * 16);
        __builtin_amdgcn_raw_buffer_store_b128(o, orsrc, ooff[j], 0, 0);
      }
    }
  };

  auto epilogue_regs = [&](Tile tc) __attribute__((always_inline)) {
    const int ty0 = tc.tyi * 16, tx0 = tc.txi * 16;
    const bool whole = ty0 + 16 <= g.MH && tx0 + 16 <= g.MW;
    const __amdgpu_buffer_rsrc_t orsrc = out_desc(tc.bimg), adrsrc = add_desc(tc.bimg);
    unsigned ooff[2], aoff[2];
#pragma unroll
    for (int mi = 0; mi < 2; ++mi) {
      const int R = wm * 64 + mi * 32 + lr, dy = R >> 4;
      const int y = ty0 + dy, x = tx0 + ((R + R_ROT * dy) & 15);
      const bool inside = whole || (y < g.MH && x < g.MW);
      const unsigned pix = (unsigned)(y * g.OW + x);
      ooff[mi] = inside ? pix * (unsigned)(g.out_cstride * 2) + lh * 16u : 0xFFFFFFF0u;
      aoff[mi] = inside ? pix * (unsigned)(g.add_cstride * 2) + lh * 16u : 0xFFFFFFF0u;
    }
    u32x4 av[2][2];
    if (g.addend) {
#pragma unroll
      for (int mi = 0; mi < 2; ++mi)
#pragma unroll
        for (int h = 0; h < 2; ++h) av[mi][h] = __builtin_amdgcn_raw_buffer_load_b128(adrsrc, aoff[mi], h * 32, 0);
    }
    if constexpr (AFFINE) {
      const float* tab = reinterpret_cast<const float*>(smem + R_OFF_PAR) + wn * 32 + 4 * lh;
#pragma unroll
      for (int q = 0; q < 4; ++q) {
        const f32x4v s4 = *reinterpret_cast<const f32x4v*>(tab + 8 * q), b4 = *reinterpret_cast<const f32x4v*>(tab + 64 + 8 * q);
#pragma unroll
        for (int mi = 0; mi < 2; ++mi)
#pragma unroll
          for (int i = 0; i < 4; ++i) acc[mi][4 * q + i] = acc[mi][4 * q + i] * s4[i] + b4[i];
      }
    }
    if (relu_first) {
#pragma unroll
      for (int mi = 0; mi < 2; ++mi)
#pragma unroll
        for (int e = 0; e < 16; ++e) acc[mi][e] = relu_bits(acc[mi][e]);
    }
    unsigned d[2][8];
#pragma unroll
    for (int mi = 0; mi < 2; ++mi)
#pragma unroll
      for (int e = 0; e < 16; e += 2) d[mi][e >> 1] = pack_bf16(acc[mi][e], acc[mi][e + 1]);
#pragma unroll
    for (int mi = 0; mi < 2; ++mi) {
#pragma unroll
      for (int q = 0; q < 4; q += 2)
#pragma unroll
        for (int w = 0; w < 2; ++w) {
          const auto r = __builtin_amdgcn_permlane32_swap(d[mi][2 * q + w], d[mi][2 * q + 2 + w], false, false);
          d[mi][2 * q + w] = r[0];
          d[mi][2 * q + 2 + w] = r[1];
        }
#pragma unroll
      for (int h = 0; h < 2; ++h) {
        u32x4 o = {d[mi][4 * h], d[mi][4 * h + 1], d[mi][4 * h + 2], d[mi][4 * h + 3]};
        if (g.addend) o = add_bf16x8(o, av[mi][h], relu_last);
        __builtin_amdgcn_raw_buffer_store_b128(o, orsrc, ooff[mi], h * 32, 0);
      }
    }
  };
  auto epilogue = [&](Tile tc, int par) __attribute__((always_inline)) {
    if constexpr (STATS) epilogue_stats(tc, par); else epilogue_regs(tc);
  };

  if constexpr (AFFINE) {
    if (tid < 128) reinterpret_cast<float*>(smem + R_OFF_PAR)[tid] = tid < 64 ? (g.scale ? g.scale[tid] : 1.f) : (bias ? bias[tid - 64] : 0.f);
  }
  const bool dyn = ticket != nullptr;
  int* const s_run = reinterpret_cast<int*>(smem + LDSB - R_RUNB);
  if (dyn) {
    if (tid == 0) {
      s_run[0] = (int)__hip_atomic_fetch_add(ticket, (unsigned)R_RUN, __ATOMIC_RELAXED, __HIP_MEMORY_SCOPE_AGENT);
      s_run[1] = (int)__hip_atomic_fetch_add(ticket, (unsigned)R_RUN, __ATOMIC_RELAXED, __HIP_MEMORY_SCOPE_AGENT);
    }
    __syncthreads();
  }
  auto tile_of = [&](int t_) { return Tile{(t_ / ttx) / tty, (t_ / ttx) % tty, t_ % ttx}; };
  int t = dyn ? s_run[0] : v, it = 0;
  int krun = 0, nrun = 0;
  int tn, kn, nn;
  unsigned pend = 0;
  int pend_slot = -1;
  auto step_walk = [&](int t_, int k_, int n_, Tile c_, int& t2, int& k2, int& n2, Tile& c2) {
    if (!dyn) {
      t2 = t_ + G; k2 = 0; n2 = 0; c2 = advance(c_);
    } else if (k_ + 1 < R_RUN && t_ + 1 < ntiles) {
      t2 = t_ + 1; k2 = k_ + 1; n2 = n_;
      c2 = c_;
      if (++c2.txi == ttx) { c2.txi = 0; if (++c2.tyi == tty) { c2.tyi = 0; ++c2.bimg; } }
    } else {
      n2 = n_ + 1; k2 = 0;
      t2 = s_run[n2 & 1];
      c2 = tile_of(t2 < ntiles ? t2 : 0);
      if (tid == 0) {
        pend = __hip_atomic_fetch_add(ticket, (unsigned)R_RUN, __ATOMIC_RELAXED, __HIP_MEMORY_SCOPE_AGENT);
        pend_slot = (n2 + 1) & 1;
      }
    }
  };
  Tile tcur = tile_of(t < ntiles ? t : 0), tprev = tcur, tprev2 = tcur, tnext;
  step_walk(t, krun, nrun, tcur, tn, kn, nn, tnext);
  if (t < ntiles) {
    const PatchSrc p0 = patch_src(tcur);
    issue_patch(p0, 0);
  }
  asm volatile("s_waitcnt vmcnt(0)" ::: "memory");
#ifdef K2R_STAMPS
  unsigned long long st_bar = 0, st_pre = 0, st_mfma = 0, st_vm = 0, st_post = 0, s0, s1;
#define K2R_STAMP(acc_) do { s1 = __builtin_readcyclecounter(); acc_ += s1 - s0; s0 = s1; } while (0)
#else
#define K2R_STAMP(acc_) do { } while (0)
#endif
  for (; t < ntiles; ++it) {
    const int buf = it & 1;
#ifdef K2R_STAMPS
    s0 = __builtin_readcyclecounter();
#endif
    asm volatile("s_waitcnt lgkmcnt(0)" ::: "memory");
    __builtin_amdgcn_s_barrier();
    asm volatile("" ::: "memory");
    K2R_STAMP(st_bar);
    if (STATS && stats && it > 1) flush_stats(tprev2, (it - 2) % 3);
    const bool more = tn < ntiles;
    const PatchSrc nxt = patch_src(tnext);
    if constexpr (ORDER == 0) {
    if (late) {
      if (it > 0) epilogue(tprev, (it - 1) % 3);
      if (more) issue_patch(nxt, buf ^ 1);
    } else if (more) {
      issue_patch(nxt, buf ^ 1);
    }
    K2R_STAMP(st_pre);
    mfma_tile(buf);
    K2R_STAMP(st_mfma);
    asm volatile("s_waitcnt vmcnt(0)" ::: "memory");
    K2R_STAMP(st_vm);
    if (!late) epilogue(tcur, it % 3);
    } else {
    if (late) {
      if (it > 0) epilogue(tprev, (it - 1) % 3);
      if (more) issue_patch(nxt, buf ^ 1);
    }
    K2R_STAMP(st_pre);
    mfma_tile(buf);
    K2R_STAMP(st_mfma);
    if (!late) {
      if (ORDER == 1 && more) issue_patch(nxt, buf ^ 1);
      epilogue(tcur, it % 3);
      if (ORDER == 2 && more) issue_patch(nxt, buf ^ 1);
    }
    asm volatile("s_waitcnt vmcnt(0)" ::: "memory");
    K2R_STAMP(st_vm);
    }
    if (dyn && tid == 0 && pend_slot >= 0 && pend_slot < 2) { s_run[pend_slot] = (int)pend; pend_slot += 2; }
    tprev2 = tprev; tprev = tcur; tcur = tnext;
    t = tn; krun = kn; nrun = nn;
    if (t < ntiles) step_walk(t, krun, nrun, tcur, tn, kn, nn, tnext);
    K2R_STAMP(st_post);
  }
#ifdef K2R_STAMPS
  if (blockIdx.x == 0 && lane == 0 && (wave == 0 || wave == 4))
    printf("K2R wave %d tiles %d: barrier %llu  pre-mfma %llu  mfma %llu  vmcnt %llu  post-mfma %llu (cycles per tile)\n", wave, it,
           st_bar / it, st_pre / it, st_mfma / it, st_vm / it, st_post / it);
#endif
  if (dyn && tid == 0) {
    asm volatile("s_waitcnt vmcnt(0)" ::: "memory");
    const unsigned old = __hip_atomic_fetch_add(ticket + 1, 1u, __ATOMIC_RELAXED, __HIP_MEMORY_SCOPE_AGENT);
    if (old == (unsigned)G - 1u) {
      __hip_atomic_store(ticket, 0u, __ATOMIC_RELAXED, __HIP_MEMORY_SCOPE_AGENT);
      __hip_atomic_store(ticket + 1, 0u, __ATOMIC_RELAXED, __HIP_MEMORY_SCOPE_AGENT);
    }
  }
  if (late && it > 0) epilogue(tprev, (it - 1) % 3);
  if (STATS && stats && it > 0) {
    __syncthreads();
    if (it > 1) flush_stats(tprev2, (it - 2) % 3);
    flush_stats(tprev, (it - 1) % 3);
  }
}

__device__ unsigned k2r_ring[2 * 1024];

unsigned* next_ticket() {
  static unsigned* base = [] {
    void* p = nullptr;
    return hipGetSymbolAddress(&p, HIP_SYMBOL(k2r_ring)) == hipSuccess ? static_cast<unsigned*>(p) : nullptr;
  }();
  static std::atomic<unsigned> n{0};
  return base ? base + 2 * (n.fetch_add(1, std::memory_order_relaxed) % 1024u) : nullptr;
}

template <int SIGN, int MODE>
void launch_k2r(const void* in, const void* wgt, const float* bias, void* out, float* stats, const ConvGeom& g, int ntiles, int grid,
                hipStream_t s) {
  static const int dynq = [] { const char* e = getenv("JSPSR_CONV_DYNQ"); return e ? atoi(e) : 0; }();
  const int forced = conv_dynq_override();
  unsigned* ticket = ((forced >= 0 ? forced : dynq) && (long long)ntiles >= 4LL * R_RUN * grid) ? next_ticket() : nullptr;
  constexpr int lds = MODE == 1 ? R_LDS_STATS : (MODE == 2 ? R_LDS_AFFINE : R_LDS_PLAIN);
  static bool attr_set = false;
  if (!attr_set) {
    (void)hipFuncSetAttribute(reinterpret_cast<const void*>(conv64_resident_kernel<SIGN, MODE>), hipFuncAttributeMaxDynamicSharedMemorySize, lds);
    attr_set = true;
  }
  hipLaunchKernelGGL((conv64_resident_kernel<SIGN, MODE>), dim3(grid), dim3(R_NTH), lds, s, static_cast<const __bf16*>(in),
                     static_cast<const __bf16*>(wgt), bias, static_cast<__bf16*>(out), stats, g, ntiles, ticket);
}

}

namespace jspsr {

bool conv64_resident_ok(const ConvGeom& g, const void* in, const void* wgt, const float* bias, const void* out) {
  static const int enabled = [] { const char* e = getenv("JSPSR_CONV_RESIDENT"); return e ? atoi(e) : 1; }();
  if (!enabled) return false;
  if (g.Cin != 64 || g.Cout != 64 || g.nty != 3 || g.ntx != 3 || g.KH != 3 || g.KW != 3) return false;
  if (g.iy_mul != 1 || g.ix_mul != 1 || g.oy_mul != 1 || g.ox_mul != 1 || g.oy_add != 0 || g.ox_add != 0) return false;
  if (g.ky0 != 0 || g.kx0 != 0 || g.kstep != 1 || g.in_affine || g.red_out) return false;
  if (g.in_cstride % 8 || g.in_coff % 8 || g.out_cstride % 8 || g.out_coff % 8) return false;
  if (!aligned16(in) || !aligned16(wgt) || !aligned16(out)) return false;
  if (g.addend && (!aligned16(g.addend) || g.add_cstride % 8)) return false;
  if ((long long)(g.IW + 20) * 20 * g.in_cstride * 2 >= 0x7fffffffLL) return false;
  if ((long long)g.OH * g.OW * g.out_cstride * 2 >= 0xF0000000LL || (long long)g.OH * g.OW * g.add_cstride * 2 >= 0xF0000000LL)
    return false;
  const long long tiles = (long long)g.B * ((g.MH + 15) / 16) * ((g.MW + 15) / 16);
  static const int min_tiles = [] { const char* e = getenv("JSPSR_CONV_RESIDENT_MIN"); return e ? atoi(e) : 512; }();
  return tiles >= min_tiles && tiles < 0x7fffffffLL;
}

int launch_conv64_resident(const void* in, const void* wgt, const float* bias, void* out, float* stats, const ConvGeom& g,
                           hipStream_t s) {
  const int ntiles = g.B * ((g.MH + 15) / 16) * ((g.MW + 15) / 16);
  static int ncu = 0;
  if (!ncu) {
    int dev = 0;
    hipDeviceProp_t p;
    if (hipGetDevice(&dev) != hipSuccess || hipGetDeviceProperties(&p, dev) != hipSuccess) return fail((int)hipErrorInvalidDevice, "conv: device query failed");
    ncu = p.multiProcessorCount > 0 ? p.multiProcessorCount : 256;
  }
  const int grid = ntiles < ncu ? ntiles : ncu;
  const int mode = stats ? 1 : ((bias || g.scale) ? 2 : 0);
  if (g.sign > 0) {
    if (mode == 0) launch_k2r<1, 0>(in, wgt, bias, out, stats, g, ntiles, grid, s);
    else if (mode == 1) launch_k2r<1, 1>(in, wgt, bias, out, stats, g, ntiles, grid, s);
    else launch_k2r<1, 2>(in, wgt, bias, out, stats, g, ntiles, grid, s);
  } else {
    if (mode == 0) launch_k2r<-1, 0>(in, wgt, bias, out, stats, g, ntiles, grid, s);
    else if (mode == 1) launch_k2r<-1, 1>(in, wgt, bias, out, stats, g, ntiles, grid, s);
    else launch_k2r<-1, 2>(in, wgt, bias, out, stats, g, ntiles, grid, s);
  }
  return check_launch("conv64_resident");
}

}
```

jspsr_amd/csrc/conv_igemm.h:

```cpp
#pragma once
#include "common.h"

namespace jspsr {

using f32x16 = __attribute__((ext_vector_type(16))) float;
using f32x4 = __attribute__((ext_vector_type(4))) float;
using bf16x8 = __attribute__((ext_vector_type(8))) __bf16;
using u16 = unsigned short;

struct ConvGeom {
  int B, IH, IW, Cin;
  int OH, OW, Cout;
  int in_cstride;
  int in_coff;
  int out_cstride;
  int out_coff;
  int MH, MW;
  int iy_mul, iy_add, ix_mul, ix_add, sign;
  int nty, ntx;
  int ky0, kx0, kstep;
  int KH, KW;
  int oy_mul, oy_add, ox_mul, ox_add;
  int relu;
  int accumulate;
  const void* addend;
  int add_cstride;
  const float* scale;
  const float* in_affine;
  int in_relu;
  FastDiv fd_ntn, fd_ttx, fd_tty;
  const void* red_x;
  int red_cstride;
  const float* red_par;
  float* red_out;
};

typedef __attribute__((address_space(3))) void* lptr_t;
typedef int i32x4 __attribute__((ext_vector_type(4)));
typedef unsigned u32x4 __attribute__((ext_vector_type(4)));
typedef float f32x2 __attribute__((ext_vector_type(2)));
typedef float f32x4v __attribute__((ext_vector_type(4)));

typedef __bf16 bf16x2 __attribute__((ext_vector_type(2)));
__device__ __forceinline__ unsigned pack_bf16(float lo, float hi) {
  const f32x2 v = {lo, hi};
  return __builtin_bit_cast(unsigned, __builtin_convertvector(v, bf16x2));
}
__device__ __forceinline__ float relu_bits(float x) { return __int_as_float(max(__float_as_int(x), 0)); }
__device__ __forceinline__ u32x4 add_bf16x8(u32x4 a, u32x4 b, bool relu) {
  u32x4 r;
#pragma unroll
  for (int i = 0; i < 4; ++i) {
    float lo = __uint_as_float(a[i] << 16) + __uint_as_float(b[i] << 16);
    float hi = __uint_as_float(a[i] & 0xffff0000u) + __uint_as_float(b[i] & 0xffff0000u);
    if (relu) { lo = relu_bits(lo); hi = relu_bits(hi); }
    r[i] = pack_bf16(lo, hi);
  }
  return r;
}


bool conv64_resident_ok(const ConvGeom& g, const void* in, const void* wgt, const float* bias, const void* out);
int launch_conv64_resident(const void* in, const void* wgt, const float* bias, void* out, float* stats, const ConvGeom& g,
                           hipStream_t s);

bool conv128_resident_ok(const ConvGeom& g, const void* in, const void* wgt, const float* bias, const void* out);
int launch_conv128_resident(const void* in, const void* wgt, const float* bias, void* out, float* stats, const ConvGeom& g, hipStream_t s);

}

template <typename T, int N>
__device__ __forceinline__ uint4 affine_relu16(const uint4& v, const float (&sc)[N], const float (&sh)[N], bool relu) {
  static_assert(N * sizeof(T) == 16, "one 16-byte chunk of channels");
  uint4 r;
  if constexpr (sizeof(T) == 4) {
    float f[4] = {__uint_as_float(v.x), __uint_as_float(v.y), __uint_as_float(v.z), __uint_as_float(v.w)};
#pragma unroll
    for (int i = 0; i < 4; ++i) {
      f[i] = f[i] * sc[i] + sh[i];
      if (relu) f[i] = fmaxf(f[i], 0.f);
    }
    r = make_uint4(__float_as_uint(f[0]), __float_as_uint(f[1]), __float_as_uint(f[2]), __float_as_uint(f[3]));
  } else {
    const unsigned w[4] = {v.x, v.y, v.z, v.w};
    unsigned o[4];
#pragma unroll
    for (int i = 0; i < 4; ++i) {
      float lo = __uint_as_float(w[i] << 16) * sc[2 * i] + sh[2 * i];
      float hi = __uint_as_float(w[i] & 0xffff0000u) * sc[2 * i + 1] + sh[2 * i + 1];
      if (relu) { lo = fmaxf(lo, 0.f); hi = fmaxf(hi, 0.f); }
      const __bf16 bl = (__bf16)lo, bh = (__bf16)hi;
      o[i] = (unsigned)__builtin_bit_cast(unsigned short, bl) | ((unsigned)__builtin_bit_cast(unsigned short, bh) << 16);
    }
    r = make_uint4(o[0], o[1], o[2], o[3]);
  }
  return r;
}
```

jspsr_amd/csrc/elementwise.hip:

```cpp
#include "common.h"

#include <cstdlib>

namespace {

using namespace jspsr;

constexpr int TX = 64, TY = 4;

template <typename T> struct V;
template <> struct V<float> { static constexpr int N = 4; };
template <> struct V<__bf16> { static constexpr int N = 8; };

template <typename T, int N>
struct Pack { T v[N]; };

template <typename T>
__device__ __forceinline__ uint4 load_raw(const T* p) { return *reinterpret_cast<const uint4*>(p); }
template <typename T>
__device__ __forceinline__ void unpack(const uint4& raw, float (&f)[V<T>::N]) {
  if constexpr (sizeof(T) == 4) {
    f[0] = __uint_as_float(raw.x); f[1] = __uint_as_float(raw.y); f[2] = __uint_as_float(raw.z); f[3] = __uint_as_float(raw.w);
  } else {
    const unsigned w[4] = {raw.x, raw.y, raw.z, raw.w};
// ... 404 lines not shown
                                                              const float* __restrict__ mean, const float* __restrict__ invstd,
                                                              const float* __restrict__ gamma, const float* __restrict__ beta,
                                                              const float* __restrict__ coef,
                                                              const unsigned char* __restrict__ mask,
                                                              T* __restrict__ dx, T* __restrict__ dres, RedGeom g) {
  constexpr int N = V<T>::N, NTEN = (RELU == 1 || RELU == 3) ? 3 : 2;
  const int C = g.C, groups = C / N;
  float mu[N], is[N], k0[N], ka[N], kb[N], ga[N], be[N];
  const int c0 = lane_map<N>(g).c;
  if (c0 < C) {
    load_param<N>(mean + c0, mu); load_param<N>(invstd + c0, is);
    load_param<N>(coef + c0, k0); load_param<N>(coef + C + c0, ka); load_param<N>(coef + 2 * C + c0, kb);
    if (RELU == 2) { load_param<N>(gamma + c0, ga); load_param<N>(beta + c0, be); }
  }
  for_pixels_mlp<T, NTEN>(
      g,
      [&](long long pix, int c, uint4 (&raw)[NTEN]) {
        raw[0] = load_raw<T>(dy + (size_t)pix * dy_cs + dy_coff + c);
        raw[1] = load_raw<T>(x + (size_t)pix * x_cs + x_coff + c);
        if constexpr (RELU == 1) raw[2] = load_raw<T>(y + (size_t)pix * y_cs + y_coff + c);
        if constexpr (RELU == 3) raw[2].x = mask[(size_t)pix * groups + c / N];
      },
      [&](long long, long long pix, int c, const uint4 (&raw)[NTEN]) {
        float d[N], xv[N], yv[N], o[N];
        unpack<T>(raw[0], d);
        unpack<T>(raw[1], xv);
        if constexpr (RELU == 1) unpack<T>(raw[2], yv);
#pragma unroll
        for (int k = 0; k < N; ++k) {
          const float xhat = (xv[k] - mu[k]) * is[k];
          const bool off = RELU == 1 ? !(yv[k] > 0.f)
                                     : (RELU == 2 ? !(ga[k] * xhat + be[k] > 0.f) : (RELU == 3 ? !((raw[2].x >> k) & 1u) : false));
          const float dz = off ? 0.f : d[k];
          d[k] = dz;
          o[k] = k0[k] * (dz - ka[k] - xhat * kb[k]);
        }
        store_vec<T>(dx + (size_t)pix * C + c, o);
        if (dres) store_vec<T>(dres + (size_t)pix * C + c, d);
      });
}

template <typename T, bool RELU>
__global__ __launch_bounds__(TX * TY) void act_bwd_kernel(const T* __restrict__ dy, int dy_cs, int dy_coff,
                                                         const T* __restrict__ y, int y_cs, int relu,
                                                         T* __restrict__ dz, int dz_cs, RedGeom g,
                                                         float* __restrict__ partial) {
  constexpr int N = V<T>::N;
  constexpr int NTEN = RELU ? 2 : 1;
  (void)relu;
  reduce_pixels_mlp<T, 1, NTEN>(
      g, partial,
      [&](long long pix, int c, uint4 (&raw)[NTEN]) {
        raw[0] = load_raw<T>(dy + (size_t)pix * dy_cs + dy_coff + c);
        if constexpr (RELU) raw[1] = load_raw<T>(y + (size_t)pix * y_cs + c);
      },
      [&](long long pix, int c, const uint4 (&raw)[NTEN], float (&acc)[1][N]) {
        float d[N], yv[N];
        unpack<T>(raw[0], d);
        if constexpr (RELU) unpack<T>(raw[1], yv);
#pragma unroll
        for (int i = 0; i < N; ++i) {
          if (RELU && !(yv[i] > 0.f)) d[i] = 0.f;
          acc[0][i] += d[i];
        }
        if (dz) store_vec<T>(dz + (size_t)pix * dz_cs + c, d);
      });
}

__global__ void sum_rows_kernel(const float* __restrict__ partial, int rows, int K, int k, int C, float* __restrict__ out) {
  const int c = blockIdx.x * (blockDim.x >> 6) + (threadIdx.x >> 6);
  if (c >= C) return;
  const double s = wave_sum_rows(partial, rows, (size_t)K * C, (size_t)k * C + c);
  if ((threadIdx.x & 63) == 0) out[c] = (float)s;
}

template <typename T>
__global__ __launch_bounds__(TX * TY) void gate_pool_kernel(const T* __restrict__ x, RedGeom g,
                                                           float* __restrict__ psum, float* __restrict__ pmax,
                                                           int* __restrict__ pidx) {
  constexpr int N = V<T>::N;
  __shared__ float rs[TY][TX * N], rm[TY][TX * N];
  __shared__ int ri[TY][TX * N];
  const int tx = threadIdx.x, ty = threadIdx.y;
  const LaneMap lm = lane_map<N>(g);
  const int c = lm.c;
  const int seg = blockIdx.x / g.chunks, chunk = blockIdx.x % g.chunks;
  float s[N], m[N];
  int idx[N];
#pragma unroll
  for (int i = 0; i < N; ++i) { s[i] = 0.f; m[i] = -INFINITY; idx[i] = 0x7fffffff; }
  const long long p0 = chunk * g.chunk_pix;
  const long long p1 = (p0 + g.chunk_pix < g.npix) ? p0 + g.chunk_pix : g.npix;
  if (c < g.C) {
    const long long step = TY * g.pl;
    long long p = p0 + ty * g.pl + lm.sub;
    auto take = [&](const uint4& raw, long long pp) {
      float f[N];
      unpack<T>(raw, f);
#pragma unroll
      for (int i = 0; i < N; ++i) {
        s[i] += f[i];
        if (f[i] > m[i]) { m[i] = f[i]; idx[i] = (int)pp; }
      }
    };
    for (; p + (PIX_FLY - 1) * step < p1; p += PIX_FLY * step) {
      uint4 raw[PIX_FLY];
#pragma unroll
      for (int u = 0; u < PIX_FLY; ++u) raw[u] = load_raw<T>(x + ((size_t)seg * g.npix + p + u * step) * g.C + c);
#pragma unroll
      for (int u = 0; u < PIX_FLY; ++u) take(raw[u], p + u * step);
    }
    for (; p < p1; p += step) take(load_raw<T>(x + ((size_t)seg * g.npix + p) * g.C + c), p);
  }
#pragma unroll
  for (int i = 0; i < N; ++i) { rs[ty][tx * N + i] = s[i]; rm[ty][tx * N + i] = m[i]; ri[ty][tx * N + i] = idx[i]; }
  __syncthreads();
  if (ty == 0 && lm.sub == 0 && c < g.C) {
#pragma unroll
    for (int i = 0; i < N; ++i) {
      float ss = 0.f, mm = -INFINITY;
      int ii = 0x7fffffff;
      for (int q = 0; q < g.pl; ++q)
#pragma unroll
      for (int y = 0; y < TY; ++y) {
        const int col = (tx + q * g.lpp) * N + i;
        ss += rs[y][col];
        const float v = rm[y][col];
        const int j = ri[y][col];
        if (v > mm || (v == mm && j < ii)) { mm = v; ii = j; }
      }
      const size_t o = (size_t)blockIdx.x * g.C + c + i;
      psum[o] = ss; pmax[o] = mm; pidx[o] = ii;
    }
  }
}

__global__ void gate_pool_finalize_kernel(const float* __restrict__ psum, const float* __restrict__ pmax,
                                          const int* __restrict__ pidx, int chunks, int C, long long npix,
                                          float* __restrict__ avg, float* __restrict__ mx, int* __restrict__ amax) {
  const int c = blockIdx.x * blockDim.x + threadIdx.x, b = blockIdx.y;
  if (c >= C) return;
  double s = 0.0;
  float m = -INFINITY;
  int ii = 0x7fffffff;
  int r = 0;
  for (; r + 8 <= chunks; r += 8) {
    float ps[8], pm[8];
    int pi[8];
#pragma unroll
    for (int k = 0; k < 8; ++k) {
      const size_t o = ((size_t)b * chunks + r + k) * C + c;
      ps[k] = psum[o]; pm[k] = pmax[o]; pi[k] = pidx[o];
    }
#pragma unroll
    for (int k = 0; k < 8; ++k) {
      s += (double)ps[k];
      if (pm[k] > m || (pm[k] == m && pi[k] < ii)) { m = pm[k]; ii = pi[k]; }
    }
  }
  for (; r < chunks; ++r) {
    const size_t o = ((size_t)b * chunks + r) * C + c;
    s += (double)psum[o];
    if (pmax[o] > m || (pmax[o] == m && pidx[o] < ii)) { m = pmax[o]; ii = pidx[o]; }
  }
  avg[(size_t)b * C + c] = (float)(s / (double)npix);
  mx[(size_t)b * C + c] = m;
  amax[(size_t)b * C + c] = ii;
}

template <typename T>
__global__ __launch_bounds__(TX * TY) void gate_scale_kernel(const T* __restrict__ x, const float* __restrict__ s,
                                                            T* __restrict__ y, RedGeom g) {
  constexpr int N = V<T>::N;
  float sv[N];
  const int c0 = lane_map<N>(g).c;
  if (c0 < g.C) load_param<N>(s + (size_t)(blockIdx.x / g.chunks) * g.C + c0, sv);
  for_pixels_mlp<T, 1>(
      g, [&](long long pix, int c, uint4 (&raw)[1]) { raw[0] = load_raw<T>(x + (size_t)pix * g.C + c); },
      [&](long long, long long pix, int c, const uint4 (&raw)[1]) {
        float f[N];
        unpack<T>(raw[0], f);
#pragma unroll
        for (int k = 0; k < N; ++k) f[k] *= sv[k];
        store_vec<T>(y + (size_t)pix * g.C + c, f);
      });
}

template <typename T>
__global__ __launch_bounds__(TX * TY) void gate_bwd_reduce_kernel(const T* __restrict__ dy, const T* __restrict__ x,
                                                                 RedGeom g, float* __restrict__ partial) {
  constexpr int N = V<T>::N;
  reduce_pixels_mlp<T, 1, 2>(
      g, partial,
      [&](long long pix, int c, uint4 (&raw)[2]) {
        raw[0] = load_raw<T>(dy + (size_t)pix * g.C + c);
        raw[1] = load_raw<T>(x + (size_t)pix * g.C + c);
      },
      [&](long long, int, const uint4 (&raw)[2], float (&acc)[1][N]) {
        float d[N], xv[N];
        unpack<T>(raw[0], d);
        unpack<T>(raw[1], xv);
#pragma unroll
        for (int i = 0; i < N; ++i) acc[0][i] += d[i] * xv[i];
      });
}

__global__ void gate_bwd_finalize_kernel(const float* __restrict__ partial, int chunks, int C, float* __restrict__ ds) {
  const int c = blockIdx.x * blockDim.x + threadIdx.x, b = blockIdx.y;
  if (c >= C) return;
  double s = 0.0;
  int r = 0;
  for (; r + 8 <= chunks; r += 8) {
    float v[8];
#pragma unroll
    for (int k = 0; k < 8; ++k) v[k] = partial[((size_t)b * chunks + r + k) * C + c];
#pragma unroll
    for (int k = 0; k < 8; ++k) s += (double)v[k];
  }
  for (; r < chunks; ++r) s += (double)partial[((size_t)b * chunks + r) * C + c];
  ds[(size_t)b * C + c] = (float)s;
}

template <typename T>
__global__ __launch_bounds__(TX * TY) void gate_bwd_apply_kernel(const T* __restrict__ dy, const float* __restrict__ s,
                                                                const float* __restrict__ davg, const float* __restrict__ dmax,
                                                                const int* __restrict__ amax, T* __restrict__ dx, RedGeom g) {
  constexpr int N = V<T>::N;
  float sv[N], da[N], dm[N];
  int am[N];
  const int c0 = lane_map<N>(g).c;
  const float inv = 1.f / (float)g.npix;
  if (c0 < g.C) {
    const size_t o = (size_t)(blockIdx.x / g.chunks) * g.C + c0;
    load_param<N>(s + o, sv); load_param<N>(davg + o, da); load_param<N>(dmax + o, dm);
#pragma unroll
    for (int k = 0; k < N; ++k) { am[k] = amax[o + k]; da[k] *= inv; }
  }
  for_pixels_mlp<T, 1>(
      g, [&](long long pix, int c, uint4 (&raw)[1]) { raw[0] = load_raw<T>(dy + (size_t)pix * g.C + c); },
      [&](long long p, long long pix, int c, const uint4 (&raw)[1]) {
        float f[N];
        unpack<T>(raw[0], f);
#pragma unroll
        for (int k = 0; k < N; ++k) f[k] = f[k] * sv[k] + da[k] + (am[k] == (int)p ? dm[k] : 0.f);
        store_vec<T>(dx + (size_t)pix * g.C + c, f);
      });
}

int ew_blocks(long long total) {
  long long b = (total + 255) / 256;
  return (int)(b < 1 ? 1 : (b > 4096 ? 4096 : b));
}

int check_c(int dtype, int C, const char* what) {
  if (dtype != JSPSR_F32 && dtype != JSPSR_BF16) return fail(JSPSR_EINVAL, "%s: bad dtype", what);
  const int vec = dtype == JSPSR_F32 ? 4 : 8;
  if (C <= 0 || C % vec) return fail(JSPSR_EINVAL, "%s: C=%d must be a multiple of %d", what, C, vec);
  return JSPSR_OK;
}

}

#define DISPATCH(dtype, CALL)                    \
  do {                                           \
    if ((dtype) == JSPSR_F32) { using T = float; CALL; } else { using T = __bf16; CALL; } \
  } while (0)

extern "C" size_t jspsr_reduce_workspace_bytes(int dtype, int C, int nseg) {
  if (C <= 0 || nseg <= 0) return 0;
  const int vec = dtype == JSPSR_F32 ? 4 : 8;
  const RedGeom g = make_red(1LL << 40, nseg, C, vec);
  const size_t rows = (size_t)nseg * g.chunks;
  return (rows * 3 + 4) * (size_t)C * sizeof(float) + 64;
}

extern "C" int jspsr_bn_forward(int dtype, const void* x, int x_cs, int x_coff, const void* res, int r_cs, int r_coff,
                                void* y, int y_cs, int y_coff, const float* gamma, const float* beta,
                                float* running_mean, float* running_var, float momentum, float eps, int training,
                                int relu, float res_scale, float* save_mean, float* save_invstd, long long npix, int C,
                                const float* ext_partial, int ext_rows, const float* res_affine, float* affine_out,
                                void* mask_out, void* workspace, jspsr_stream_t stream) {
  if (int e = check_c(dtype, C, "bn_forward")) return e;
  if (!x || (!y && !affine_out) || !gamma || !beta || !save_mean || !save_invstd || !workspace || npix <= 0)
    return fail(JSPSR_EINVAL, "bn_forward: null pointer or empty tensor");
  if (res_affine && !res) return fail(JSPSR_EINVAL, "bn_forward: res_affine without a residual operand");
  if (mask_out && (!res || !relu || !y)) return fail(JSPSR_EINVAL, "bn_forward: mask_out needs an output with residual and ReLU");
  if (!training && (!running_mean || !running_var)) return fail(JSPSR_EINVAL, "bn_forward: eval mode needs running stats");
  const int vec = dtype == JSPSR_F32 ? 4 : 8;
  if (x_cs % vec || x_coff % vec || y_cs % vec || y_coff % vec || (res && (r_cs % vec || r_coff % vec)))
    return fail(JSPSR_EINVAL, "bn_forward: channel pitches/offsets must be multiples of %d", vec);
  hipStream_t s = static_cast<hipStream_t>(stream);
  float* ws = static_cast<float*>(workspace);
  float* scale = affine_out ? affine_out : ws;
  float* shift = affine_out ? affine_out + C : ws + C;
  float* partial = ws + 2 * C;
  int rows = 0;
  if (training && ext_partial) {
    if (ext_rows <= 0) return fail(JSPSR_EINVAL, "bn_forward: ext_rows must be positive");
    rows = ext_rows < 256 ? ext_rows : 256;
    if (ext_rows > 256) {
      hipLaunchKernelGGL(fold_rows_kernel, dim3(rows, (2 * C + 255) / 256), dim3(256), 0, s, ext_partial, ext_rows, 2 * C, rows, partial);
      if (int e = check_launch("bn_fold_rows")) return e;
    } else {
      (void)hipMemcpyAsync(partial, ext_partial, (size_t)ext_rows * 2 * C * sizeof(float), hipMemcpyDeviceToDevice, s);
    }
  } else if (training) {
    const RedGeom g = make_red(npix, 1, C, vec);
    rows = g.chunks;
    DISPATCH(dtype, hipLaunchKernelGGL(bn_stats_kernel<T>, red_grid(g, vec), dim3(TX, TY), 0, s,
                                       static_cast<const T*>(x), x_cs, x_coff, g, partial));
    if (int e = check_launch("bn_stats")) return e;
  }
  hipLaunchKernelGGL(bn_finalize_kernel, dim3((C + 3) / 4), dim3(256), 0, s, partial, rows, C, npix, gamma, beta,
                     running_mean, running_var, momentum, eps, training, save_mean, save_invstd, scale, shift);
  if (int e = check_launch("bn_finalize")) return e;
  if (!y) return JSPSR_OK;
  const RedGeom ga = make_red(npix, 1, C, vec);
#define BN_APPLY(R, M) DISPATCH(dtype, hipLaunchKernelGGL((bn_apply_kernel<T, R, M>), red_grid(ga, vec), dim3(TX, TY), 0, s,       \
                                     static_cast<const T*>(x), x_cs, x_coff, static_cast<const T*>(res), r_cs, r_coff,        \
                                     static_cast<T*>(y), y_cs, y_coff, scale, shift, res_affine, res_scale, relu,             \
                                     static_cast<unsigned char*>(mask_out), ga))
  if (mask_out) { BN_APPLY(true, true); } else if (res) { BN_APPLY(true, false); } else { BN_APPLY(false, false); }
#undef BN_APPLY
  return check_launch("bn_apply");
}

__global__ void bn_reduce_params_kernel(const float* __restrict__ gamma, const float* __restrict__ beta, const float* __restrict__ mean,
                                        const float* __restrict__ invstd, int C, float* __restrict__ par) {
  const int c = blockIdx.x * blockDim.x + threadIdx.x;
  if (c >= C) return;
  const float a = gamma[c] * invstd[c];
  par[c] = a;
  par[C + c] = beta[c] - a * mean[c];
  par[2 * C + c] = invstd[c];
  par[3 * C + c] = -mean[c] * invstd[c];
}

extern "C" size_t jspsr_bn_mask_bytes(int dtype, long long npix, int C) {
  const int vec = dtype == JSPSR_F32 ? 4 : 8;
  if (npix <= 0 || C <= 0 || C % vec) return 0;
  return (size_t)npix * (size_t)(C / vec);
}

extern "C" int jspsr_bn_reduce_params(const float* gamma, const float* beta, const float* save_mean, const float* save_invstd, int C,
                                      float* par, jspsr_stream_t stream) {
  if (!gamma || !beta || !save_mean || !save_invstd || !par || C <= 0) return fail(JSPSR_EINVAL, "bn_reduce_params: bad arguments");
  hipLaunchKernelGGL(bn_reduce_params_kernel, dim3((C + 255) / 256), dim3(256), 0, static_cast<hipStream_t>(stream), gamma, beta,
                     save_mean, save_invstd, C, par);
  return check_launch("bn_reduce_params");
}

extern "C" int jspsr_bn_backward(int dtype, const void* dy, int dy_cs, int dy_coff, const void* y, int y_cs, int y_coff,
                                 const void* x, int x_cs, int x_coff, const float* gamma, const float* beta, const float* save_mean,
                                 const float* save_invstd, int training, int relu, float res_scale, void* dx, void* dres,
                                 float* dgamma, float* dbeta, int accumulate, long long npix, int C, void* workspace,
                                 const float* ext_partial, int ext_rows, const void* mask, jspsr_stream_t stream) {
  if (int e = check_c(dtype, C, "bn_backward")) return e;
  if (!dy || !x || !gamma || !save_mean || !save_invstd || !dx || !dgamma || !dbeta || !workspace || npix <= 0 ||
      (relu == 1 && !y && !mask) || (relu == 2 && !beta) || relu < 0 || relu > 2)
    return fail(JSPSR_EINVAL, "bn_backward: null pointer, empty tensor or bad relu mode");
  const int vec = dtype == JSPSR_F32 ? 4 : 8;
  if (dy_cs % vec || dy_coff % vec || x_cs % vec || x_coff % vec || (relu == 1 && !mask && (y_cs % vec || y_coff % vec)))
    return fail(JSPSR_EINVAL, "bn_backward: channel pitches/offsets must be multiples of %d", vec);
  hipStream_t s = static_cast<hipStream_t>(stream);
  float* ws = static_cast<float*>(workspace);
  float* coef = ws;
  float* partial = ws + 3 * C;
  const RedGeom g = make_red(npix, 1, C, vec);
  const unsigned char* mk = relu == 1 ? static_cast<const unsigned char*>(mask) : nullptr;
  const int mode = (relu == 1 && mk) ? 3 : relu;
  const bool premask = relu == 1 && dres && !ext_partial;
#define BN_BWD_REDUCE(R, D) DISPATCH(dtype, hipLaunchKernelGGL((bn_bwd_reduce_kernel<T, R, D>), red_grid(g, vec), dim3(TX, TY), 0, s, \
                                     static_cast<const T*>(dy), dy_cs, dy_coff, static_cast<const T*>(y), y_cs, y_coff,     \
                                     static_cast<const T*>(x), x_cs, x_coff, save_mean, save_invstd, gamma, beta, mk,        \
                                     static_cast<T*>(dres), g, partial))
  int rows = g.chunks;
  if (ext_partial) {
    if (ext_rows <= 0) return fail(JSPSR_EINVAL, "bn_backward: ext_rows must be positive");
    if (ext_rows > 1024) {
      rows = g.chunks < 1024 ? (g.chunks > 0 ? g.chunks : 1) : 1024;
      hipLaunchKernelGGL(fold_rows_kernel, dim3(rows, (2 * C + 255) / 256), dim3(256), 0, s, ext_partial, ext_rows, 2 * C, rows, partial);
      if (int e = check_launch("bn_fold_rows")) return e;
    } else {
      partial = const_cast<float*>(ext_partial);
      rows = ext_rows;
    }
  } else {
    if (mode == 0) { BN_BWD_REDUCE(0, false); }
    else if (mode == 2) { BN_BWD_REDUCE(2, false); }
    else if (mode == 1) { if (premask) { BN_BWD_REDUCE(1, true); } else { BN_BWD_REDUCE(1, false); } }
    else { if (premask) { BN_BWD_REDUCE(3, true); } else { BN_BWD_REDUCE(3, false); } }
    if (int e = check_launch("bn_bwd_reduce")) return e;
  }
#undef BN_BWD_REDUCE
  hipLaunchKernelGGL(bn_bwd_finalize_kernel, dim3((C + 3) / 4), dim3(256), 0, s, partial, rows, C, npix, gamma,
                     save_invstd, training, res_scale, accumulate, dgamma, dbeta, coef);
  if (int e = check_launch("bn_bwd_finalize")) return e;
#define BN_BWD_APPLY(R, DY, CS, OFF, DRES) DISPATCH(dtype, hipLaunchKernelGGL((bn_bwd_apply_kernel<T, R>), red_grid(g, vec), dim3(TX, TY), 0, s, \
                                     static_cast<const T*>(DY), CS, OFF, static_cast<const T*>(y), y_cs, y_coff,            \
                                     static_cast<const T*>(x), x_cs, x_coff, save_mean, save_invstd, gamma, beta, coef, mk, \
                                     static_cast<T*>(dx), static_cast<T*>(DRES), g))
  if (premask) { BN_BWD_APPLY(0, dres, C, 0, nullptr); }
  else if (mode == 0) { BN_BWD_APPLY(0, dy, dy_cs, dy_coff, dres); }
  else if (mode == 1) { BN_BWD_APPLY(1, dy, dy_cs, dy_coff, dres); }
  else if (mode == 2) { BN_BWD_APPLY(2, dy, dy_cs, dy_coff, dres); }
  else { BN_BWD_APPLY(3, dy, dy_cs, dy_coff, dres); }
#undef BN_BWD_APPLY
  return check_launch("bn_bwd_apply");
}

extern "C" int jspsr_bn_fold(const float* gamma, const float* beta, const float* running_mean, const float* running_var,
                             float eps, float res_scale, int C, float* scale, float* shift, jspsr_stream_t stream) {
  if (!gamma || !beta || !running_mean || !running_var || !scale || !shift || C <= 0)
    return fail(JSPSR_EINVAL, "bn_fold: bad arguments");
  hipLaunchKernelGGL(bn_fold_kernel, dim3((C + 255) / 256), dim3(256), 0, static_cast<hipStream_t>(stream), gamma, beta,
                     running_mean, running_var, eps, res_scale, C, scale, shift);
  return check_launch("bn_fold");
}

extern "C" int jspsr_act_backward(int dtype, const void* dy, int dy_cs, int dy_coff, const void* y, int y_cs, int relu,
                                  void* dz, int dz_cs, float* dbias, long long npix, int C, void* workspace,
                                  jspsr_stream_t stream) {
  if (int e = check_c(dtype, C, "act_backward")) return e;
  if (!dy || (relu && !y) || !workspace || npix <= 0) return fail(JSPSR_EINVAL, "act_backward: null pointer or empty tensor");
  const int vec = dtype == JSPSR_F32 ? 4 : 8;
  if (dy_cs % vec || dy_coff % vec || (dz && dz_cs % vec) || (relu && (y_cs % vec || y_cs < C)))
    return fail(JSPSR_EINVAL, "act_backward: bad pitch");
  hipStream_t s = static_cast<hipStream_t>(stream);
  float* partial = static_cast<float*>(workspace);
  const RedGeom g = make_red(npix, 1, C, vec);
#define ACT_BWD(R) DISPATCH(dtype, hipLaunchKernelGGL((act_bwd_kernel<T, R>), red_grid(g, vec), dim3(TX, TY), 0, s, static_cast<const T*>(dy), \
                                     dy_cs, dy_coff, static_cast<const T*>(y), y_cs, relu, static_cast<T*>(dz), dz_cs, g, partial))
  if (relu) { ACT_BWD(true); } else { ACT_BWD(false); }
#undef ACT_BWD
  if (int e = check_launch("act_backward")) return e;
  if (dbias) {
    hipLaunchKernelGGL(sum_rows_kernel, dim3((C + 3) / 4), dim3(256), 0, s, partial, g.chunks, 1, 0, C, dbias);
    return check_launch("act_backward_bias");
  }
  return JSPSR_OK;
}

extern "C" int jspsr_gate_pool(int dtype, const void* x, int B, long long npix, int C, float* avg, float* mx, int* amax,
                               void* workspace, jspsr_stream_t stream) {
  if (int e = check_c(dtype, C, "gate_pool")) return e;
  if (!x || !avg || !mx || !amax || !workspace || B <= 0 || npix <= 0 || npix > 0x7fffffffLL)
    return fail(JSPSR_EINVAL, "gate_pool: bad arguments");
  const int vec = dtype == JSPSR_F32 ? 4 : 8;
  hipStream_t s = static_cast<hipStream_t>(stream);
  const RedGeom g = make_red(npix, B, C, vec);
  const size_t rows = (size_t)B * g.chunks;
  float* psum = static_cast<float*>(workspace);
  float* pmax = psum + rows * C;
  int* pidx = reinterpret_cast<int*>(pmax + rows * C);
  DISPATCH(dtype, hipLaunchKernelGGL(gate_pool_kernel<T>, red_grid(g, vec), dim3(TX, TY), 0, s, static_cast<const T*>(x), g,
                                     psum, pmax, pidx));
  if (int e = check_launch("gate_pool")) return e;
  hipLaunchKernelGGL(gate_pool_finalize_kernel, dim3((C + 255) / 256, B), dim3(256), 0, s, psum, pmax, pidx, g.chunks, C,
                     npix, avg, mx, amax);
  return check_launch("gate_pool_finalize");
}

extern "C" int jspsr_gate_scale(int dtype, const void* x, const float* s_, void* y, int B, long long npix, int C,
                                jspsr_stream_t stream) {
  if (int e = check_c(dtype, C, "gate_scale")) return e;
  if (!x || !s_ || !y || B <= 0 || npix <= 0) return fail(JSPSR_EINVAL, "gate_scale: bad arguments");
  const int vec = dtype == JSPSR_F32 ? 4 : 8;
  hipStream_t s = static_cast<hipStream_t>(stream);
  const RedGeom g = make_red(npix, B, C, vec);
  DISPATCH(dtype, hipLaunchKernelGGL(gate_scale_kernel<T>, red_grid(g, vec), dim3(TX, TY), 0, s,
                                     static_cast<const T*>(x), s_, static_cast<T*>(y), g));
  return check_launch("gate_scale");
}

extern "C" int jspsr_gate_backward_reduce(int dtype, const void* dy, const void* x, float* ds, int B, long long npix, int C,
                                          void* workspace, jspsr_stream_t stream) {
  if (int e = check_c(dtype, C, "gate_backward_reduce")) return e;
  if (!dy || !x || !ds || !workspace || B <= 0 || npix <= 0) return fail(JSPSR_EINVAL, "gate_backward_reduce: bad arguments");
  const int vec = dtype == JSPSR_F32 ? 4 : 8;
  hipStream_t s = static_cast<hipStream_t>(stream);
  const RedGeom g = make_red(npix, B, C, vec);
  float* partial = static_cast<float*>(workspace);
  DISPATCH(dtype, hipLaunchKernelGGL(gate_bwd_reduce_kernel<T>, red_grid(g, vec), dim3(TX, TY), 0, s,
                                     static_cast<const T*>(dy), static_cast<const T*>(x), g, partial));
  if (int e = check_launch("gate_backward_reduce")) return e;
  hipLaunchKernelGGL(gate_bwd_finalize_kernel, dim3((C + 255) / 256, B), dim3(256), 0, s, partial, g.chunks, C, ds);
  return check_launch("gate_backward_finalize");
}

extern "C" int jspsr_gate_backward_apply(int dtype, const void* dy, const float* s_, const float* davg, const float* dmax,
                                         const int* amax, void* dx, int B, long long npix, int C, jspsr_stream_t stream) {
  if (int e = check_c(dtype, C, "gate_backward_apply")) return e;
  if (!dy || !s_ || !davg || !dmax || !amax || !dx || B <= 0 || npix <= 0)
    return fail(JSPSR_EINVAL, "gate_backward_apply: bad arguments");
  const int vec = dtype == JSPSR_F32 ? 4 : 8;
  hipStream_t s = static_cast<hipStream_t>(stream);
  const RedGeom g = make_red(npix, B, C, vec);
  DISPATCH(dtype, hipLaunchKernelGGL(gate_bwd_apply_kernel<T>, red_grid(g, vec), dim3(TX, TY), 0, s,
                                     static_cast<const T*>(dy), s_, davg, dmax, amax, static_cast<T*>(dx), g));
  return check_launch("gate_backward_apply");
}

template <typename T>
__global__ __launch_bounds__(256) void nchw_to_nhwc_kernel(const float* __restrict__ src, T* __restrict__ dst, int C, long long HW,
                                                          long long npix, int Cpad) {
  constexpr int N = V<T>::N;
  for (long long p = blockIdx.x * 256LL + threadIdx.x; p < npix; p += (long long)gridDim.x * 256) {
    const long long b = p / HW, q = p - b * HW;
    const float* s = src + (size_t)b * C * HW + q;
    T* d = dst + (size_t)p * Cpad;
    for (int c0 = 0; c0 < Cpad; c0 += N) {
      float f[N];
#pragma unroll
      for (int i = 0; i < N; ++i) f[i] = c0 + i < C ? s[(size_t)(c0 + i) * HW] : 0.f;
      store_vec<T>(d + c0, f);
    }
  }
}

extern "C" int jspsr_nchw_to_nhwc(int dtype, const float* src, void* dst, int B, int C, int H, int W, int c_pad,
                                  jspsr_stream_t stream) {
  if (dtype != JSPSR_F32 && dtype != JSPSR_BF16) return fail(JSPSR_EINVAL, "nchw_to_nhwc: dtype must be JSPSR_F32 or JSPSR_BF16");
  const int vec = dtype == JSPSR_F32 ? 4 : 8;
  if (!src || !dst || B <= 0 || C <= 0 || H <= 0 || W <= 0 || c_pad < C || c_pad % vec)
    return fail(JSPSR_EINVAL, "nchw_to_nhwc: bad arguments (c_pad must be a multiple of %d and >= C)", vec);
  if (!aligned4(src) || !aligned16(dst)) return fail(JSPSR_EALIGN, "nchw_to_nhwc: src must be 4-byte, dst 16-byte aligned");
  const long long HW = (long long)H * W, npix = HW * B;
  const long long want = (npix + 255) / 256;
  const int blocks = (int)(want > 8192 ? 8192 : want);
  hipStream_t s = static_cast<hipStream_t>(stream);
  DISPATCH(dtype, hipLaunchKernelGGL(nchw_to_nhwc_kernel<T>, dim3(blocks), dim3(256), 0, s, src, static_cast<T*>(dst), C, HW, npix, c_pad));
  return check_launch("nchw_to_nhwc");
}

constexpr int GM_T = 256;

__global__ __launch_bounds__(GM_T) void gate_mlp_fwd_kernel(const float* __restrict__ avg, const float* __restrict__ mx,
                                                           const float* __restrict__ w1, const float* __restrict__ w2, int C, int Ch,
                                                           float* __restrict__ s, float* __restrict__ hid) {
  extern __shared__ float gm_lds[];
  const int b = blockIdx.x, tid = threadIdx.x, wave = tid >> 6, lane = tid & 63;
  const float* a = avg + (size_t)b * C;
  const float* m = mx + (size_t)b * C;
  for (int j = wave; j < Ch; j += GM_T / 64) {
    const float* w = w1 + (size_t)j * C;
    float da = 0.f, dm = 0.f;
    for (int c = lane; c < C; c += 64) { const float wv = w[c]; da += wv * a[c]; dm += wv * m[c]; }
#pragma unroll
    for (int d = 32; d > 0; d >>= 1) { da += __shfl_xor(da, d, 64); dm += __shfl_xor(dm, d, 64); }
    if (lane == 0) {
      const float ha = fmaxf(da, 0.f), hm = fmaxf(dm, 0.f);
      hid[((size_t)b * 2 + 0) * Ch + j] = ha;
      hid[((size_t)b * 2 + 1) * Ch + j] = hm;
      gm_lds[j] = ha + hm;
    }
  }
  __syncthreads();
  for (int c = tid; c < C; c += GM_T) {
    const float* w = w2 + (size_t)c * Ch;
    float z = 0.f;
    for (int j = 0; j < Ch; ++j) z += w[j] * gm_lds[j];
    s[(size_t)b * C + c] = 1.f / (1.f + expf(-z));
  }
}

__global__ __launch_bounds__(GM_T) void gate_mlp_bwd_kernel(const float* __restrict__ ds, const float* __restrict__ s,
                                                           const float* __restrict__ hid, const float* __restrict__ w1,
                                                           const float* __restrict__ w2, int C, int Ch, float* __restrict__ davg,
                                                           float* __restrict__ dmax, float* __restrict__ dzs, float* __restrict__ dhs) {
  extern __shared__ float gm_lds[];
  float* dz = gm_lds;
  float* dh = gm_lds + C;
  const int b = blockIdx.x, tid = threadIdx.x, wave = tid >> 6, lane = tid & 63;
  for (int c = tid; c < C; c += GM_T) {
    const float sv = s[(size_t)b * C + c], v = ds[(size_t)b * C + c] * sv * (1.f - sv);
    dz[c] = v;
    dzs[(size_t)b * C + c] = v;
  }
  __syncthreads();
  for (int j = wave; j < Ch; j += GM_T / 64) {
    float acc = 0.f;
    for (int c = lane; c < C; c += 64) acc += w2[(size_t)c * Ch + j] * dz[c];
#pragma unroll
    for (int d = 32; d > 0; d >>= 1) acc += __shfl_xor(acc, d, 64);
    if (lane == 0) {
      const float da = hid[((size_t)b * 2 + 0) * Ch + j] > 0.f ? acc : 0.f, dm = hid[((size_t)b * 2 + 1) * Ch + j] > 0.f ? acc : 0.f;
      dh[j] = da; dh[Ch + j] = dm;
      dhs[((size_t)b * 2 + 0) * Ch + j] = da;
      dhs[((size_t)b * 2 + 1) * Ch + j] = dm;
    }
  }
  __syncthreads();
  for (int c = tid; c < C; c += GM_T) {
    float ga = 0.f, gm = 0.f;
    for (int j = 0; j < Ch; ++j) { const float wv = w1[(size_t)j * C + c]; ga += wv * dh[j]; gm += wv * dh[Ch + j]; }
    davg[(size_t)b * C + c] = ga;
    dmax[(size_t)b * C + c] = gm;
  }
}

__global__ __launch_bounds__(GM_T) void gate_mlp_wgrad_kernel(const float* __restrict__ dzs, const float* __restrict__ dhs,
                                                             const float* __restrict__ hid, const float* __restrict__ avg,
                                                             const float* __restrict__ mx, int B, int C, int Ch,
                                                             float* __restrict__ dw1, float* __restrict__ dw2) {
  const long long n = (long long)C * Ch;
  for (long long i = blockIdx.x * (long long)GM_T + threadIdx.x; i < 2 * n; i += (long long)gridDim.x * GM_T) {
    if (i < n) {
// ... 47 lines not shown
```

Measured before the change: 35.45 Mpixel/s.

## Fold input BatchNorm affine+ReLU into resident 64/128-channel conv kernels

Lets the resident conv64 (stats form) and conv128 (forward, no bias) kernels accept a per-channel input affine+ReLU. Input patches are loaded into registers, transformed, and stored to LDS, replacing the direct buffer-to-LDS DMA. These convs previously fell back to the generic patch kernel and now stay on the faster resident path. A second change reads the BN partial-stat buffer directly instead of copying it first. The register staging adds VGPR pressure and VALU work on the load path, which could hurt overlap.

```diff
diff --git a/jspsr_amd/csrc/conv.hip b/jspsr_amd/csrc/conv.hip
--- a/jspsr_amd/csrc/conv.hip
+++ b/jspsr_amd/csrc/conv.hip
@@ -987,7 +987,7 @@
   constexpr int BKT = NCH * Elem<T>::EPC;
   if constexpr (sizeof(T) == 2)
   {
-    if (conv64_resident_ok(g, in, wgt, bias, out)) return launch_conv64_resident(in, wgt, bias, out, stats, g, s);
+    if (conv64_resident_ok(g, in, wgt, bias, out, stats)) return launch_conv64_resident(in, wgt, bias, out, stats, g, s);
     if (conv128_resident_ok(g, in, wgt, bias, out)) return launch_conv128_resident(in, wgt, bias, out, stats, g, s);
   }
   if ((!no_patch || g.in_affine) && g.iy_mul == 1 && g.ix_mul == 1 && g.nty >= 1 && g.ntx >= 1 && g.nty <= 3 && g.ntx <= 3 &&
diff --git a/jspsr_amd/csrc/conv128.hip b/jspsr_amd/csrc/conv128.hip
--- a/jspsr_amd/csrc/conv128.hip
+++ b/jspsr_amd/csrc/conv128.hip
@@ -91,10 +91,12 @@
 struct QTile { int bimg, tyi, txi; };
 struct QSrc { i32x4 desc; __amdgpu_buffer_rsrc_t rsrc; int oy0, ox0; bool interior; };
 
-template <int SIGN, int MODE, int KH>
+template <int SIGN, int MODE, int KH, bool INAFF>
 __device__ __forceinline__ void conv128_body(const __bf16* __restrict__ in, const __bf16* __restrict__ wgt, const float* __restrict__ bias,
                                              __bf16* __restrict__ out, float* __restrict__ stats, const ConvGeom& g, int ntiles, unsigned* __restrict__ ticket, char* smem) {
   constexpr bool STATS = MODE == 1, AFFINE = MODE == 2;
+  constexpr int DMA_MODE = INAFF ? 3 : K2Q_DMA_MODE;
+  static_assert(!INAFF || SIGN > 0, "the input transform exists on the forward walk only");
   const int tid = threadIdx.x, wave = __builtin_amdgcn_readfirstlane(tid >> 6), lane = tid & 63;
   const int cg = wave & 1;
   const int n = lane & 15, q = lane >> 4;
@@ -171,6 +173,22 @@
     src = (unsigned)(p.ox0 + c.px) < (unsigned)g.IW ? src : 0xFFFFFFF0u;
     return src;
   };
+  float isc[8], ish[8];
+  if constexpr (INAFF) {
+    const float* ap = g.in_affine + (swz16 >> 4) * 8;
+#pragma unroll
+    for (int e = 0; e < 8; e += 4) {
+      const f32x4 a4 = *reinterpret_cast<const f32x4*>(ap + e), b4 = *reinterpret_cast<const f32x4*>(ap + 128 + e);
+#pragma unroll
+      for (int j = 0; j < 4; ++j) { isc[e + j] = a4[j]; ish[e + j] = b4[j]; }
+    }
+  }
+  const bool irelu = g.in_relu != 0;
+  auto xform = [&](const u32x4& v, unsigned src) __attribute__((always_inline)) {
+    const uint4 r = affine_relu16<__bf16>(make_uint4(v[0], v[1], v[2], v[3]), isc, ish, irelu);
+    const bool ok = src != 0xFFFFFFF0u;
+    return u32x4{ok ? r.x : 0u, ok ? r.y : 0u, ok ? r.z : 0u, ok ? r.w : 0u};
+  };
   auto piece_dst = [&](unsigned bufoff, int i) __attribute__((always_inline)) {
 #ifdef K2Q_LAB_TODUMP
     return (unsigned)Q_OFF_DUMP;
@@ -227,6 +245,7 @@
     i32x4 a[Q_LAH];
     constexpr int NSTG = (K2Q_LD_DIST + K2Q_LD_EVERY - 1) / K2Q_LD_EVERY;
     u32x4 stg[NSTG];
+    unsigned stgsrc[NSTG];
     static_for<0, Q_NK + Q_LAH>([&](auto K) __attribute__((always_inline)) {
       constexpr int k = decltype(K)::value;
       if constexpr (k >= Q_LAH) {
@@ -242,18 +261,21 @@
         constexpr int ty = SIGN > 0 ? tap / 3 : 2 - tap / 3, tx = SIGN > 0 ? tap % 3 : 2 - tap % 3;
         constexpr int R = r + ty;
         a[k % Q_LAH] = *reinterpret_cast<lds_frag_t>((abase[R & 3][tx] ^ (unsigned)(s * 64)) + (unsigned)((R >> 2) * Q_ROWS4));
-        if constexpr (K2Q_DMA_MODE == 1 && k % K2Q_DMA_EVERY == 2 && k / K2Q_DMA_EVERY < Q_NP) issue_piece(nxt, nbufoff, k / K2Q_DMA_EVERY);
+        if constexpr (DMA_MODE == 1 && k % K2Q_DMA_EVERY == 2 && k / K2Q_DMA_EVERY < Q_NP) issue_piece(nxt, nbufoff, k / K2Q_DMA_EVERY);
         if constexpr (!STATS && k == 1) prefetch_addend(tc);
-        if constexpr (K2Q_DMA_MODE == 3) {
+        if constexpr (DMA_MODE == 3) {
           constexpr int LD = K2Q_LD_EVERY, WD = K2Q_LD_DIST;
           static_assert(2 + LD * (Q_NP - 1) + WD < Q_NK, "the last piece is written inside the loop");
           if constexpr (k >= 2 + WD && (k - 2 - WD) % LD == 0 && (k - 2 - WD) / LD < Q_NP) {
             constexpr int j = (k - 2 - WD) / LD;
-            *reinterpret_cast<u32x4*>(smem + piece_dst(nbufoff, j) + lane * 16) = stg[j % NSTG];
+            if constexpr (INAFF) *reinterpret_cast<u32x4*>(smem + piece_dst(nbufoff, j) + lane * 16) = xform(stg[j % NSTG], stgsrc[j % NSTG]);
+            else *reinterpret_cast<u32x4*>(smem + piece_dst(nbufoff, j) + lane * 16) = stg[j % NSTG];
           }
           if constexpr (k >= 2 && (k - 2) % LD == 0 && (k - 2) / LD < Q_NP) {
             constexpr int j = (k - 2) / LD;
-            stg[j % NSTG] = __builtin_amdgcn_raw_buffer_load_b128(nxt.rsrc, piece_src(nxt, piece_xy(j)), 0, 0);
+            const unsigned src = piece_src(nxt, piece_xy(j));
+            stg[j % NSTG] = __builtin_amdgcn_raw_buffer_load_b128(nxt.rsrc, src, 0, 0);
+            stgsrc[j % NSTG] = src;
           }
         }
       }
@@ -402,8 +424,17 @@
   unsigned bufoff = 0;
   if (t < ntiles) {
     const QSrc p0 = patch_src(tcur, true);
-#pragma unroll
-    for (int i = 0; i < Q_NP; ++i) issue_piece(p0, 0u, i);
+    if constexpr (INAFF) {
+#pragma unroll
+      for (int i = 0; i < Q_NP; ++i) {
+        const unsigned src = piece_src(p0, piece_xy(i));
+        const u32x4 pv = __builtin_amdgcn_raw_buffer_load_b128(p0.rsrc, src, 0, 0);
+        *reinterpret_cast<u32x4*>(smem + piece_dst(0u, i) + lane * 16) = xform(pv, src);
+      }
+    } else {
+#pragma unroll
+      for (int i = 0; i < Q_NP; ++i) issue_piece(p0, 0u, i);
+    }
   }
   __builtin_amdgcn_s_waitcnt(0x0F70);
   asm volatile("" ::: "memory");
@@ -444,7 +475,7 @@
     }
     const bool more = tn < ntiles;
     const QSrc nxt = patch_src(tnext, more);
-    if (K2Q_DMA_MODE == 0) {
+    if (DMA_MODE == 0) {
 #pragma unroll
       for (int i = 0; i < Q_NP; ++i) issue_piece(nxt, bufoff ^ Q_BUF1, i);
     }
@@ -485,13 +516,13 @@
   }
 }
 
-template <int SIGN, int MODE>
+template <int SIGN, int MODE, bool INAFF>
 __global__ __launch_bounds__(Q_NTH) __attribute__((amdgpu_waves_per_eu(1, 1))) void conv128_resident_kernel(
     const __bf16* __restrict__ in, const __bf16* __restrict__ wgt, const float* __restrict__ bias, __bf16* __restrict__ out,
     float* __restrict__ stats, ConvGeom g, int ntiles, unsigned* __restrict__ ticket) {
   extern __shared__ __attribute__((aligned(128))) char smem[];
-  if (__builtin_amdgcn_readfirstlane(threadIdx.x >> 7) == 0) conv128_body<SIGN, MODE, 0>(in, wgt, bias, out, stats, g, ntiles, ticket, smem);
-  else conv128_body<SIGN, MODE, 1>(in, wgt, bias, out, stats, g, ntiles, ticket, smem);
+  if (__builtin_amdgcn_readfirstlane(threadIdx.x >> 7) == 0) conv128_body<SIGN, MODE, 0, INAFF>(in, wgt, bias, out, stats, g, ntiles, ticket, smem);
+  else conv128_body<SIGN, MODE, 1, INAFF>(in, wgt, bias, out, stats, g, ntiles, ticket, smem);
 }
 
 __device__ unsigned k2q_ring[2 * 1024];
@@ -505,17 +536,17 @@
   return base ? base + 2 * (n.fetch_add(1, std::memory_order_relaxed) % 1024u) : nullptr;
 }
 
-template <int SIGN, int MODE>
+template <int SIGN, int MODE, bool INAFF = false>
 void launch_k2q(const void* in, const void* wgt, const float* bias, void* out, float* stats, const ConvGeom& g, int ntiles, int grid, hipStream_t s) {
   static bool attr_set = false;
   if (!attr_set) {
-    (void)hipFuncSetAttribute(reinterpret_cast<const void*>(conv128_resident_kernel<SIGN, MODE>), hipFuncAttributeMaxDynamicSharedMemorySize, Q_LDS);
+    (void)hipFuncSetAttribute(reinterpret_cast<const void*>(conv128_resident_kernel<SIGN, MODE, INAFF>), hipFuncAttributeMaxDynamicSharedMemorySize, Q_LDS);
     attr_set = true;
   }
   static const int dynq = [] { const char* e = getenv("JSPSR_CONV_DYNQ128"); return e ? atoi(e) : 0; }();
   const int forced = conv_dynq_override();
   unsigned* ticket = ((forced >= 0 ? forced : dynq) && (long long)ntiles >= 4LL * Q_RUN * grid) ? next_ticket() : nullptr;
-  hipLaunchKernelGGL((conv128_resident_kernel<SIGN, MODE>), dim3(grid), dim3(Q_NTH), Q_LDS, s, static_cast<const __bf16*>(in),
+  hipLaunchKernelGGL((conv128_resident_kernel<SIGN, MODE, INAFF>), dim3(grid), dim3(Q_NTH), Q_LDS, s, static_cast<const __bf16*>(in),
                      static_cast<const __bf16*>(wgt), bias, static_cast<__bf16*>(out), stats, g, ntiles, ticket);
 }
 
@@ -528,7 +559,11 @@
   if (!enabled) return false;
   if (g.Cin != 128 || g.Cout != 128 || g.nty != 3 || g.ntx != 3 || g.KH != 3 || g.KW != 3) return false;
   if (g.iy_mul != 1 || g.ix_mul != 1 || g.oy_mul != 1 || g.ox_mul != 1 || g.oy_add != 0 || g.ox_add != 0) return false;
-  if (g.ky0 != 0 || g.kx0 != 0 || g.kstep != 1 || g.in_affine || g.red_out) return false;
+  if (g.ky0 != 0 || g.kx0 != 0 || g.kstep != 1 || g.red_out) return false;
+  if (g.in_affine) {
+    static const int in_aff = [] { const char* e = getenv("JSPSR_CONV_RESIDENT_AFFINE"); return e ? atoi(e) : 1; }();
+    if (!in_aff || g.sign < 0 || bias || g.scale || !aligned16(g.in_affine)) return false;
+  }
   if (bias && !aligned4(bias)) return false;
   if (g.sign < 0 && (bias || g.scale)) return false;
   if (g.in_cstride % 8 || g.in_coff % 8 || g.out_cstride % 8 || g.out_coff % 8) return false;
@@ -557,7 +592,11 @@
     fprintf(stderr, "K2q sign %d B %d %dx%d in pitch %d off %d out pitch %d off %d addend %d (pitch %d) relu %d stats %d in %p out %p\n", g.sign, g.B,
             g.MH, g.MW, g.in_cstride, g.in_coff, g.out_cstride, g.out_coff, g.addend != nullptr, g.add_cstride, g.relu, stats != nullptr, in, out);
   const int mode = stats ? 1 : ((bias || g.scale) ? 2 : 0);
-  if (g.sign > 0) {
+  if (g.in_affine) {
+    if (g.sign < 0 || mode == 2) return fail(JSPSR_EINVAL, "conv128_resident: in_affine exists on the forward walk without bias / scale only");
+    if (mode == 0) launch_k2q<1, 0, true>(in, wgt, bias, out, stats, g, ntiles, grid, s);
+    else launch_k2q<1, 1, true>(in, wgt, bias, out, stats, g, ntiles, grid, s);
+  } else if (g.sign > 0) {
     if (mode == 0) launch_k2q<1, 0>(in, wgt, bias, out, stats, g, ntiles, grid, s);
     else if (mode == 1) launch_k2q<1, 1>(in, wgt, bias, out, stats, g, ntiles, grid, s);
     else launch_k2q<1, 2>(in, wgt, bias, out, stats, g, ntiles, grid, s);
diff --git a/jspsr_amd/csrc/conv64.hip b/jspsr_amd/csrc/conv64.hip
--- a/jspsr_amd/csrc/conv64.hip
+++ b/jspsr_amd/csrc/conv64.hip
@@ -25,6 +25,9 @@
 #else
 constexpr int early_pieces(bool stats) { return stats ? 8 : 6; }
 #endif
+#ifndef K2R_EARLY_INAFF
+#define K2R_EARLY_INAFF 8
+#endif
 constexpr int R_PATCHB = R_PIECES * R_PIECEB + 16;
 constexpr int R_SCRP = 80;
 constexpr int R_SCRB = 64 * R_SCRP;
@@ -32,6 +35,9 @@
 constexpr int R_OFF_RED = R_OFF_SCR + 8 * R_SCRB;
 constexpr int R_RUNB = 16;
 constexpr int R_LDS_STATS = R_OFF_RED + 3 * 4 * 2 * 64 * 4 + R_RUNB;
+constexpr int R_OFF_INAFF = R_LDS_STATS - R_RUNB;
+constexpr int R_LDS_STATS_INAFF = R_OFF_INAFF + 2 * 64 * 4 + R_RUNB;
+static_assert(R_LDS_STATS_INAFF <= 163840, "LDS of one CU");
 constexpr int R_LDS_PLAIN = 2 * R_PATCHB + R_RUNB;
 constexpr int R_OFF_PAR = 2 * R_PATCHB;
 constexpr int R_LDS_AFFINE = R_OFF_PAR + 2 * 64 * 4 + R_RUNB;
@@ -43,15 +49,15 @@
 constexpr int NK = 72, LA = K2R_LA;
 
 struct Tile { int bimg, tyi, txi; };
-struct PatchSrc { i32x4 desc; int oy0, ox0; bool interior; };
-
-template <int SIGN, int MODE>
+struct PatchSrc { i32x4 desc; __amdgpu_buffer_rsrc_t rsrc; int oy0, ox0; bool interior; };
+
+template <int SIGN, int MODE, bool INAFF>
 __global__ __launch_bounds__(R_NTH) void conv64_resident_kernel(const __bf16* __restrict__ in, const __bf16* __restrict__ wgt,
                                                                   const float* __restrict__ bias, __bf16* __restrict__ out,
                                                                   float* __restrict__ stats, ConvGeom g, int ntiles,
                                                                   unsigned* __restrict__ ticket) {
   constexpr bool STATS = MODE == 1, AFFINE = MODE == 2;
-  constexpr int LDSB = MODE == 1 ? R_LDS_STATS : (MODE == 2 ? R_LDS_AFFINE : R_LDS_PLAIN);
+  constexpr int LDSB = INAFF ? R_LDS_STATS_INAFF : (MODE == 1 ? R_LDS_STATS : (MODE == 2 ? R_LDS_AFFINE : R_LDS_PLAIN));
   extern __shared__ __attribute__((aligned(128))) char smem[];
   const int tid = threadIdx.x, wave = __builtin_amdgcn_readfirstlane(tid >> 6), lane = tid & 63;
   const int wm = (wave >> 1) & 3, wn = wave & 1;
@@ -61,7 +67,8 @@
   const unsigned lds0 = (unsigned)(size_t)(lptr_t)smem;
   const int v = xcd_contiguous(blockIdx.x, G);
   const bool late = wave >= 4;
-  constexpr int ORDER = order_of(STATS), R_PE = early_pieces(STATS), R_PL = (R_PIECES - 4 * R_PE + 3) / 4;
+  static_assert(!INAFF || (SIGN > 0 && STATS), "the input transform exists in the statistics form of the forward walk only");
+  constexpr int ORDER = order_of(STATS), R_PE = INAFF ? K2R_EARLY_INAFF : early_pieces(STATS), R_PL = (R_PIECES - 4 * R_PE + 3) / 4;
   constexpr int R_PIT = R_PE > R_PL ? R_PE : R_PL;
 
   bf16x8 breg[9][4];
@@ -94,7 +101,7 @@
   for (int i = 0; i < R_PIT; ++i) {
     const int P = (piece0 + 4 * i) * R_PPP + lpix;
     const int py = P / R_PW, px = P - py * R_PW;
-    dsrc[i] = (lp16 < 128 && P < R_NPIX) ? (unsigned)((py * g.IW + px) * pix_bytes + lp16) : 0xFFFFFFF0u;
+    dsrc[i] = (!INAFF && lp16 < 128 && P < R_NPIX) ? (unsigned)((py * g.IW + px) * pix_bytes + lp16) : 0xFFFFFFF0u;
   }
   auto patch_src = [&](Tile tc) {
     PatchSrc p;
@@ -104,21 +111,70 @@
     const unsigned long long b64 = reinterpret_cast<unsigned long long>(in) + (opix0 * g.in_cstride + g.in_coff) * 2;
     p.desc = i32x4{(int)(unsigned)b64, (int)((unsigned)(b64 >> 32) & 0xffffu), (int)0xFFFFFF00u, 0x00020000};
     p.interior = p.oy0 >= 0 && p.ox0 >= 0 && p.oy0 + R_PW <= g.IH && p.ox0 + R_PW <= g.IW;
+    if constexpr (INAFF) p.rsrc = __builtin_amdgcn_make_buffer_rsrc(reinterpret_cast<char*>(b64), 0, 0xFFFFFF00u, 0x00020000);
     return p;
   };
+  auto piece_src = [&](const PatchSrc& p, int i) __attribute__((always_inline)) {
+    unsigned src = dsrc[i];
+    if (!p.interior) {
+      int lpix_ = lpix;
+      asm volatile("" : "+v"(lpix_));
+      const int P = (piece0 + 4 * i) * R_PPP + lpix_;
+      const int py = (int)(__umul24(P, 3641) >> 16), px = P - (int)__umul24(py, R_PW);
+      const bool in_img = (unsigned)(p.oy0 + py) < (unsigned)g.IH && (unsigned)(p.ox0 + px) < (unsigned)g.IW;
+      src = in_img ? src : 0xFFFFFFF0u;
+    }
+    return src;
+  };
+  u32x4 stg[INAFF ? R_PIT : 1];
+  const bool irelu = g.in_relu != 0;
+  struct PieceLane { unsigned src; bool store, in_img; int slot, lane; };
+  auto piece_lane = [&](const PatchSrc& p, int i) __attribute__((always_inline)) {
+    PieceLane c;
+    c.lane = lane;
+    asm volatile("" : "+v"(c.lane));
+    const int lp = (int)(__umul24(c.lane, 3641) >> 15);
+    c.slot = c.lane - 9 * lp;
+    const int P = (piece0 * R_PPP + lp) + 4 * R_PPP * i;
+    const int py = (int)(__umul24(P, 3641) >> 16), px = P - (int)__umul24(py, R_PW);
+    c.store = c.slot < 8 && c.lane < 63 && P < R_NPIX;
+    c.in_img = (unsigned)(p.oy0 + py) < (unsigned)g.IH && (unsigned)(p.ox0 + px) < (unsigned)g.IW;
+    c.src = (c.store && c.in_img) ? __umul24(__umul24(py, g.IW) + (unsigned)px, pix_bytes) + (unsigned)c.slot * 16u : 0xFFFFFFF0u;
+    return c;
+  };
+  auto load_patch = [&](const PatchSrc& p) __attribute__((always_inline)) {
+#pragma unroll
+    for (int i = 0; i < R_PIT; ++i)
+      if (i < npiece && piece0 + 4 * i < R_PIECES)
+        stg[INAFF ? i : 0] = __builtin_amdgcn_raw_buffer_load_b128(p.rsrc, piece_lane(p, i).src, 0, 0);
+  };
+  auto store_patch = [&](const PatchSrc& p, int buf) __attribute__((always_inline)) {
+    const PieceLane c0 = piece_lane(p, 0);
+    float isc[8], ish[8];
+    const float* ap = reinterpret_cast<const float*>(smem + R_OFF_INAFF) + (c0.slot & 7) * 8;
+#pragma unroll
+    for (int e = 0; e < 8; e += 4) {
+      const f32x4v a4 = *reinterpret_cast<const f32x4v*>(ap + e), b4 = *reinterpret_cast<const f32x4v*>(ap + 64 + e);
+#pragma unroll
+      for (int j = 0; j < 4; ++j) { isc[e + j] = a4[j]; ish[e + j] = b4[j]; }
+    }
+    char* const dst0 = smem + buf * R_PATCHB + piece0 * R_PIECEB + c0.lane * 16;
+#pragma unroll
+    for (int i = 0; i < R_PIT; ++i)
+      if (i < npiece && piece0 + 4 * i < R_PIECES) {
+        const PieceLane c = piece_lane(p, i);
+        const u32x4 v = stg[INAFF ? i : 0];
+        const uint4 r = affine_relu16<__bf16>(make_uint4(v[0], v[1], v[2], v[3]), isc, ish, irelu);
+        const u32x4 o = {c.in_img ? r.x : 0u, c.in_img ? r.y : 0u, c.in_img ? r.z : 0u, c.in_img ? r.w : 0u};
+        if (c.store) *reinterpret_cast<u32x4*>(dst0 + 4 * i * R_PIECEB) = o;
+      }
+  };
   auto issue_patch = [&](const PatchSrc& p, int buf) __attribute__((always_inline)) {
+    if constexpr (INAFF) { load_patch(p); return; }
 #pragma unroll
     for (int i = 0; i < R_PIT; ++i) {
       if (i < npiece && piece0 + 4 * i < R_PIECES) {
-        unsigned src = dsrc[i];
-        if (!p.interior) {
-          int lpix_ = lpix;
-          asm volatile("" : "+v"(lpix_));
-          const int P = (piece0 + 4 * i) * R_PPP + lpix_;
-          const int py = (int)(__umul24(P, 3641) >> 16), px = P - (int)__umul24(py, R_PW);
-          const bool in_img = (unsigned)(p.oy0 + py) < (unsigned)g.IH && (unsigned)(p.ox0 + px) < (unsigned)g.IW;
-          src = in_img ? src : 0xFFFFFFF0u;
-        }
+        const unsigned src = piece_src(p, i);
         const unsigned dst = lds0 + buf * R_PATCHB + (piece0 + 4 * i) * R_PIECEB;
         asm volatile("s_mov_b32 m0, %0\n\ts_nop 0\n\tbuffer_load_dwordx4 %1, %2, 0 offen lds" : : "s"(dst), "v"(src), "s"(p.desc));
       }
@@ -163,9 +219,7 @@
   };
 
   const bool relu_first = g.relu && !g.addend, relu_last = g.relu && g.addend;
-  char* const scr = smem + R_OFF_SCR + wave * R_SCRB;
   float* const red = reinterpret_cast<float*>(smem + R_OFF_RED);
-  const int ncol = wn * 32 + lr;
   const int tty8 = (g.MH + 7) >> 3;
 
   auto flush_stats = [&](Tile tc, int par) __attribute__((always_inline)) {
@@ -190,6 +244,10 @@
 
   auto epilogue_stats = [&](Tile tc, int par) __attribute__((always_inline)) {
     const int ty0 = tc.tyi * 16, tx0 = tc.txi * 16;
+    int le = lane;
+    if constexpr (INAFF) asm volatile("" : "+v"(le));
+    const int lr = le & 31, lh = le >> 5, ncol = wn * 32 + lr;
+    char* const scr = smem + R_OFF_SCR + wave * R_SCRB;
     const bool whole = ty0 + 16 <= g.MH && tx0 + 16 <= g.MW;
     if (stats) {
       float s = 0.f, q = 0.f;
@@ -237,7 +295,7 @@
         *reinterpret_cast<__bf16*>(scr + row * R_SCRP + lr * 2) = (__bf16)o;
       }
     asm volatile("s_waitcnt lgkmcnt(0)" ::: "memory");
-    const int c16 = lane & 3, prow = lane >> 2;
+    const int c16 = le & 3, prow = le >> 2;
     const __amdgpu_buffer_rsrc_t orsrc = out_desc(tc.bimg), adrsrc = add_desc(tc.bimg);
     unsigned ooff[4], aoff[4];
 #pragma unroll
@@ -369,11 +427,22 @@
   };
   Tile tcur = tile_of(t < ntiles ? t : 0), tprev = tcur, tprev2 = tcur, tnext;
   step_walk(t, krun, nrun, tcur, tn, kn, nn, tnext);
+  if constexpr (INAFF) {
+    if (tid < 128) reinterpret_cast<float*>(smem + R_OFF_INAFF)[tid] = g.in_affine[tid];
+    __syncthreads();
+  }
   if (t < ntiles) {
     const PatchSrc p0 = patch_src(tcur);
     issue_patch(p0, 0);
+    if constexpr (INAFF) store_patch(p0, 0);
   }
   asm volatile("s_waitcnt vmcnt(0)" ::: "memory");
+  auto load_ahead = [&]() __attribute__((always_inline)) {
+    if constexpr (INAFF) {
+      if (late && t < ntiles && tn < ntiles) load_patch(patch_src(tnext));
+    }
+  };
+  load_ahead();
 #ifdef K2R_STAMPS
   unsigned long long st_bar = 0, st_pre = 0, st_mfma = 0, st_vm = 0, st_post = 0, s0, s1;
 #define K2R_STAMP(acc_) do { s1 = __builtin_readcyclecounter(); acc_ += s1 - s0; s0 = s1; } while (0)
@@ -392,7 +461,21 @@
     if (STATS && stats && it > 1) flush_stats(tprev2, (it - 2) % 3);
     const bool more = tn < ntiles;
     const PatchSrc nxt = patch_src(tnext);
-    if constexpr (ORDER == 0) {
+    if constexpr (INAFF) {
+    if (late) {
+      if (it > 0) epilogue(tprev, (it - 1) % 3);
+      if (more) store_patch(nxt, buf ^ 1);
+    }
+    K2R_STAMP(st_pre);
+    mfma_tile(buf);
+    K2R_STAMP(st_mfma);
+    if (!late) {
+      if (more) load_patch(nxt);
+      epilogue(tcur, it % 3);
+      if (more) store_patch(nxt, buf ^ 1);
+    }
+    K2R_STAMP(st_vm);
+    } else if constexpr (ORDER == 0) {
     if (late) {
       if (it > 0) epilogue(tprev, (it - 1) % 3);
       if (more) issue_patch(nxt, buf ^ 1);
@@ -425,6 +508,7 @@
     tprev2 = tprev; tprev = tcur; tcur = tnext;
     t = tn; krun = kn; nrun = nn;
     if (t < ntiles) step_walk(t, krun, nrun, tcur, tn, kn, nn, tnext);
+    load_ahead();
     K2R_STAMP(st_post);
   }
 #ifdef K2R_STAMPS
@@ -459,19 +543,19 @@
   return base ? base + 2 * (n.fetch_add(1, std::memory_order_relaxed) % 1024u) : nullptr;
 }
 
-template <int SIGN, int MODE>
+template <int SIGN, int MODE, bool INAFF = false>
 void launch_k2r(const void* in, const void* wgt, const float* bias, void* out, float* stats, const ConvGeom& g, int ntiles, int grid,
                 hipStream_t s) {
   static const int dynq = [] { const char* e = getenv("JSPSR_CONV_DYNQ"); return e ? atoi(e) : 0; }();
   const int forced = conv_dynq_override();
   unsigned* ticket = ((forced >= 0 ? forced : dynq) && (long long)ntiles >= 4LL * R_RUN * grid) ? next_ticket() : nullptr;
-  constexpr int lds = MODE == 1 ? R_LDS_STATS : (MODE == 2 ? R_LDS_AFFINE : R_LDS_PLAIN);
+  constexpr int lds = INAFF ? R_LDS_STATS_INAFF : (MODE == 1 ? R_LDS_STATS : (MODE == 2 ? R_LDS_AFFINE : R_LDS_PLAIN));
   static bool attr_set = false;
   if (!attr_set) {
-    (void)hipFuncSetAttribute(reinterpret_cast<const void*>(conv64_resident_kernel<SIGN, MODE>), hipFuncAttributeMaxDynamicSharedMemorySize, lds);
+    (void)hipFuncSetAttribute(reinterpret_cast<const void*>(conv64_resident_kernel<SIGN, MODE, INAFF>), hipFuncAttributeMaxDynamicSharedMemorySize, lds);
     attr_set = true;
   }
-  hipLaunchKernelGGL((conv64_resident_kernel<SIGN, MODE>), dim3(grid), dim3(R_NTH), lds, s, static_cast<const __bf16*>(in),
+  hipLaunchKernelGGL((conv64_resident_kernel<SIGN, MODE, INAFF>), dim3(grid), dim3(R_NTH), lds, s, static_cast<const __bf16*>(in),
                      static_cast<const __bf16*>(wgt), bias, static_cast<__bf16*>(out), stats, g, ntiles, ticket);
 }
 
@@ -479,12 +563,16 @@
 
 namespace jspsr {
 
-bool conv64_resident_ok(const ConvGeom& g, const void* in, const void* wgt, const float* bias, const void* out) {
+bool conv64_resident_ok(const ConvGeom& g, const void* in, const void* wgt, const float* bias, const void* out, const float* stats) {
   static const int enabled = [] { const char* e = getenv("JSPSR_CONV_RESIDENT"); return e ? atoi(e) : 1; }();
   if (!enabled) return false;
   if (g.Cin != 64 || g.Cout != 64 || g.nty != 3 || g.ntx != 3 || g.KH != 3 || g.KW != 3) return false;
   if (g.iy_mul != 1 || g.ix_mul != 1 || g.oy_mul != 1 || g.ox_mul != 1 || g.oy_add != 0 || g.ox_add != 0) return false;
-  if (g.ky0 != 0 || g.kx0 != 0 || g.kstep != 1 || g.in_affine || g.red_out) return false;
+  if (g.ky0 != 0 || g.kx0 != 0 || g.kstep != 1 || g.red_out) return false;
+  if (g.in_affine) {
+    static const int in_aff = [] { const char* e = getenv("JSPSR_CONV_RESIDENT_AFFINE"); return e ? atoi(e) : 1; }();
+    if (!in_aff || g.sign < 0 || !stats || !aligned16(g.in_affine)) return false;
+  }
   if (g.in_cstride % 8 || g.in_coff % 8 || g.out_cstride % 8 || g.out_coff % 8) return false;
   if (!aligned16(in) || !aligned16(wgt) || !aligned16(out)) return false;
   if (g.addend && (!aligned16(g.addend) || g.add_cstride % 8)) return false;
@@ -508,7 +596,10 @@
   }
   const int grid = ntiles < ncu ? ntiles : ncu;
   const int mode = stats ? 1 : ((bias || g.scale) ? 2 : 0);
-  if (g.sign > 0) {
+  if (g.in_affine) {
+    if (g.sign < 0 || mode != 1) return fail(JSPSR_EINVAL, "conv64_resident: in_affine exists in the statistics form of the forward walk only");
+    launch_k2r<1, 1, true>(in, wgt, bias, out, stats, g, ntiles, grid, s);
+  } else if (g.sign > 0) {
     if (mode == 0) launch_k2r<1, 0>(in, wgt, bias, out, stats, g, ntiles, grid, s);
     else if (mode == 1) launch_k2r<1, 1>(in, wgt, bias, out, stats, g, ntiles, grid, s);
     else launch_k2r<1, 2>(in, wgt, bias, out, stats, g, ntiles, grid, s);
diff --git a/jspsr_amd/csrc/conv_igemm.h b/jspsr_amd/csrc/conv_igemm.h
--- a/jspsr_amd/csrc/conv_igemm.h
+++ b/jspsr_amd/csrc/conv_igemm.h
@@ -60,7 +60,7 @@
 }
 
 
-bool conv64_resident_ok(const ConvGeom& g, const void* in, const void* wgt, const float* bias, const void* out);
+bool conv64_resident_ok(const ConvGeom& g, const void* in, const void* wgt, const float* bias, const void* out, const float* stats);
 int launch_conv64_resident(const void* in, const void* wgt, const float* bias, void* out, float* stats, const ConvGeom& g,
                            hipStream_t s);
 
diff --git a/jspsr_amd/csrc/elementwise.hip b/jspsr_amd/csrc/elementwise.hip
--- a/jspsr_amd/csrc/elementwise.hip
+++ b/jspsr_amd/csrc/elementwise.hip
@@ -730,7 +730,7 @@
       hipLaunchKernelGGL(fold_rows_kernel, dim3(rows, (2 * C + 255) / 256), dim3(256), 0, s, ext_partial, ext_rows, 2 * C, rows, partial);
       if (int e = check_launch("bn_fold_rows")) return e;
     } else {
-      (void)hipMemcpyAsync(partial, ext_partial, (size_t)ext_rows * 2 * C * sizeof(float), hipMemcpyDeviceToDevice, s);
+      partial = const_cast<float*>(ext_partial);
     }
   } else if (training) {
     const RedGeom g = make_red(npix, 1, C, vec);
```

Result: no change. 35.13 Mpixel/s (-0.9%).
